# OpenGene/repaq

Measured on AMD Instinct MI355X. Metric: raw FASTQ MB/s encode+decode, higher is better.
Workload: dtype u8; 1 GPU; configs[2]: synthetic NovaSeq PE150 two files (-i/-I), 2 x 4.01 GB FASTQ (fqgen profile 1, 11200000 pairs, seed 3, N 20 ppm), -k 1000, encode + decode; chunks_per_gpu=3360, parity=unchecked (checked with --full)

## Files before the change

repaq_amd/csrc/dec/pos_lists.h:

```cpp
#pragma once
#define POS2_SEG 1024u
#define POS2_SEG_BIG 2048u
#define POS2_CELL 1024u
typedef uint16_t plist_t;
__device__ __forceinline__ uint32_t plist_pos(uint32_t e, uint32_t w0) { return e == 0xFFFFFFFFu ? e : w0 + ((e - w0) & 0xFFFFu); }
struct PosSrc { const uint8_t* sp; uint32_t slen; uint8_t q; };
__device__ __forceinline__ PosSrc pos_src_of(const uint8_t* __restrict__ img, const DChunk& d, const DevHeader* __restrict__ D, uint32_t jj, DecStatus* st) {
    PosSrc s; s.sp = nullptr; s.slen = 0; s.q = 0;
    const uint32_t nn = D->n_normal, hf = D->flags; const uint8_t* cp = img + d.off;
    if (jj == nn) { if (hf & H_N_POS) { s.sp = cp + d.o_npos; s.slen = d.npos_size; s.q = (uint8_t)'N'; } return s; }
    if (jj > nn || jj >= NPOS_SLOT || (hf & H_DONT_QUAL) || !(hf & H_QUAL_BY_COL)) return s;
    if (4ull * nn > d.qual_size) { if (st && lane_id() == 0) atomicOr(&st->err, (uint32_t)DE_CORRUPT); return s; }
    const uint8_t* qp = cp + d.o_qual; uint64_t off = 4ull * nn;
    for (uint32_t i = 0; i < jj; i++) off += ld_u32(qp + 4 * i);
    const uint32_t sl = ld_u32(qp + 4 * jj);
    if (off + sl > d.qual_size) { if (st && lane_id() == 0) atomicOr(&st->err, (uint32_t)DE_CORRUPT); return s; }
    s.sp = qp + off; s.slen = sl; s.q = D->normal[jj];
    return s;
}
__device__ __forceinline__ void pos_lane_adv_cnt(const PosFront& f, uint32_t slen, uint32_t i0, uint32_t st, int& adv, int& cnt) {
    adv = 0; cnt = 0;
#pragma unroll
    for (int k = 0; k < 4; k++) {
        const uint32_t b0 = f.bt[k]; const bool valid = i0 + (uint32_t)k < slen;
        const uint32_t b1 = (uint32_t)(f.v >> (8 * (k + 1))) & 0xFFu, b2 = (uint32_t)(f.v >> (8 * (k + 2))) & 0xFFu, b3 = (uint32_t)(f.v >> (8 * (k + 3))) & 0xFFu;
        if (valid && st == 0) {
            if ((b0 & 0x80u) == 0) { adv += (int)b0 + 1; cnt++; }
            else if ((b0 & 0x40u) == 0) { adv += (int)(((b0 & 0x3Fu) << 8) | b1) + 1; cnt++; }
            else if ((b0 & 0x20u) == 0) { adv += (int)(b0 & 0x1Fu) + 1; cnt += (int)(b0 & 0x1Fu) + 1; }
            else { adv += (int)(((b0 & 0x1Fu) << 24) | (b1 << 16) | (b2 << 8) | b3) + 1; cnt++; }
        }
        if (valid) st = fn_apply(f.fn[k], st);
    }
}
__device__ __forceinline__ int sel4(const int (&v)[4], uint32_t t) { return t == 0 ? v[0] : (t == 1 ? v[1] : (t == 2 ? v[2] : v[3])); }
__device__ __forceinline__ void pos_lane_adv_cnt4(const PosFront& f, uint32_t slen, uint32_t i0, int (&adv)[4], int (&cnt)[4]) {
    const uint32_t nv = i0 >= slen ? 0u : (slen - i0 < 4u ? slen - i0 : 4u);
    int ca[4], cc[4]; uint32_t tl[4];
#pragma unroll
    for (int k = 0; k < 4; k++) {
        const uint32_t b0 = f.bt[k];
        const uint32_t b1 = (uint32_t)(f.v >> (8 * (k + 1))) & 0xFFu, b2 = (uint32_t)(f.v >> (8 * (k + 2))) & 0xFFu, b3 = (uint32_t)(f.v >> (8 * (k + 3))) & 0xFFu;
        if ((b0 & 0x80u) == 0) { ca[k] = (int)b0 + 1; cc[k] = 1; tl[k] = 1; }
        else if ((b0 & 0x40u) == 0) { ca[k] = (int)(((b0 & 0x3Fu) << 8) | b1) + 1; cc[k] = 1; tl[k] = 2; }
        else if ((b0 & 0x20u) == 0) { ca[k] = (int)(b0 & 0x1Fu) + 1; cc[k] = ca[k]; tl[k] = 1; }
        else { ca[k] = (int)(((b0 & 0x1Fu) << 24) | (b1 << 16) | (b2 << 8) | b3) + 1; cc[k] = 1; tl[k] = 4; }
    }
#pragma unroll
    for (int k = 2; k >= 0; k--) {
        const uint32_t nx = (uint32_t)k + tl[k];
        if (nx < nv) { const int a_ = nx == 1u ? ca[1] : (nx == 2u ? ca[2] : ca[3]), c_ = nx == 1u ? cc[1] : (nx == 2u ? cc[2] : cc[3]); ca[k] += a_; cc[k] += c_; }
    }
#pragma unroll
    for (int s = 0; s < 4; s++) { const bool on = (uint32_t)s < nv; adv[s] = on ? ca[s] : 0; cnt[s] = on ? cc[s] : 0; }
}
#define POS_ADV_MAX 0x3FFFFFFFull
__device__ __forceinline__ int pos_adv_sat(int v) { return v > (int)POS_ADV_MAX ? (int)POS_ADV_MAX : v; }
__global__ void k_dec_pos_sum2(const uint8_t* __restrict__ img, const DChunk* __restrict__ CH, const DevHeader* __restrict__ D,
                               uint8_t* __restrict__ segF, int* __restrict__ segA, uint32_t* __restrict__ segN, uint32_t maxseg, DecStatus* st, uint64_t img_bytes, uint32_t jj0, uint32_t nstr,
                               uint32_t segb) {
    const uint32_t g = blockIdx.x * (blockDim.x >> 6) + (uint32_t)wave_id(), jj = jj0 + blockIdx.y, c = blockIdx.z; const int l = lane_id();
            const uint8_t* lim = img + img_bytes;
    const DChunk d = CH[c];
    const PosSrc s = pos_src_of(img, d, D, jj, g == 0 ? st : nullptr);
    if (g == 0 && l == 0) segN[(size_t)c * nstr + jj] = (s.slen + segb - 1) / segb;
    const uint32_t b0 = g * segb; if (b0 >= s.slen) return;
    const uint32_t b1 = b0 + segb < s.slen ? b0 + segb : s.slen;
    uint32_t Fcum = POS_ID; int a[4] = { 0, 0, 0, 0 }, n[4] = { 0, 0, 0, 0 };
    PosStep nxt = pos_fetch(s.sp, s.slen, b0 + 4u * (uint32_t)l, lim);
    for (uint32_t base = b0; base < b1; base += 256u) {
        const uint32_t i0 = base + 4u * (uint32_t)l;
        const PosStep w = nxt;
        if (base + 256u < b1) nxt = pos_fetch(s.sp, s.slen, i0 + 256u, lim);
        const PosFront f = pos_front(w, s.sp, s.slen, i0, l);
        const uint32_t Fex = wave_shr1(f.Fin, POS_ID);
        const uint32_t G = fn_compose(Fcum, Fex);
        int la[4], lc[4]; pos_lane_adv_cnt4(f, s.slen, i0, la, lc);
#pragma unroll
        for (int e = 0; e < 4; e++) { const uint32_t t_ = fn_apply(G, e); a[e] += sel4(la, t_); n[e] += sel4(lc, t_); }
        Fcum = fn_compose(Fcum, wave_last(f.Fin));
    }
#pragma unroll
    for (int e = 0; e < 4; e++) { const unsigned long long w64 = wave_sum<unsigned long long>((unsigned long long)(uint32_t)a[e]); a[e] = (int)(w64 > POS_ADV_MAX ? POS_ADV_MAX : w64);
            n[e] = wave_sum(n[e]); }
    if (l == 0) { const size_t idx = ((size_t)c * nstr + jj) * maxseg + g; segF[idx] = (uint8_t)fn_pack8(Fcum);
#pragma unroll
                  for (int e = 0; e < 4; e++) { segA[8 * idx + e] = a[e]; segA[8 * idx + 4 + e] = n[e]; } }
}
struct PosLink { uint32_t F; int a[4], n[4]; };
__device__ __forceinline__ PosLink poslink_then(const PosLink& x, const PosLink& y) {
    PosLink r; r.F = fn_compose(x.F, y.F);
#pragma unroll
    for (int s = 0; s < 4; s++) { const uint32_t t = fn_apply(x.F, s); r.a[s] = pos_adv_sat(x.a[s] + sel4(y.a, t)); r.n[s] = x.n[s] + sel4(y.n, t); }
    return r;
}
__device__ __forceinline__ PosLink poslink_shfl_up(const PosLink& v, unsigned dd) {
    PosLink u; u.F = __shfl_up(v.F, dd);
#pragma unroll
    for (int s = 0; s < 4; s++) { u.a[s] = __shfl_up(v.a[s], dd); u.n[s] = __shfl_up(v.n[s], dd); }
    return u;
}
__global__ void k_dec_pos_link2(const uint8_t* __restrict__ segF, const int* __restrict__ segA, const uint32_t* __restrict__ segN, uint8_t* __restrict__ segS,
        int* __restrict__ segP,
                                uint32_t* __restrict__ segK, uint32_t* __restrict__ nent, uint32_t maxseg, uint32_t n_streams,
                                const DChunk* __restrict__ CH, uint32_t nstr, DecStatus* st) {
    const uint32_t t = blockIdx.x * (blockDim.x >> 6) + (uint32_t)wave_id(); if (t >= n_streams) return;
    const int l = lane_id(); const uint32_t n = segN[t];
    uint32_t cs = 0; int cp = -1; uint32_t ck = 0;
    for (uint32_t base = 0; base < n; base += 64) {
        const uint32_t g = base + (uint32_t)l; const size_t idx = (size_t)t * maxseg + g;
        PosLink me; me.F = POS_ID;
#pragma unroll
        for (int s = 0; s < 4; s++) { me.a[s] = 0; me.n[s] = 0; }
        if (g < n) { me.F = fn_unpack8(segF[idx]);
#pragma unroll
                     for (int s = 0; s < 4; s++) { me.a[s] = segA[8 * idx + s]; me.n[s] = segA[8 * idx + 4 + s]; } }
        PosLink inc = me;
#pragma unroll
        for (int dd = 1; dd < 64; dd <<= 1) { const PosLink up = poslink_shfl_up(inc, (unsigned)dd); if (l >= dd) inc = poslink_then(up, inc); }
        PosLink ex = poslink_shfl_up(inc, 1u);
        if (l == 0) { ex.F = POS_ID;
#pragma unroll
                      for (int s = 0; s < 4; s++) { ex.a[s] = 0; ex.n[s] = 0; } }
        if (g < n) { segS[idx] = (uint8_t)(fn_apply(ex.F, cs)); segP[idx] = pos_adv_sat(cp + sel4(ex.a, cs)); segK[idx] = ck + (uint32_t)sel4(ex.n, cs); }
        const uint32_t Fl = wave_last(inc.F); int al[4], nl[4];
#pragma unroll
        for (int s = 0; s < 4; s++) { al[s] = wave_last(inc.a[s]); nl[s] = wave_last(inc.n[s]); }
        cp = pos_adv_sat(cp + sel4(al, cs)); ck += (uint32_t)sel4(nl, cs); cs = fn_apply(Fl, cs);
    }
    if (l == 0) {
        nent[t] = ck;
        const unsigned long long ext = CH[t / nstr].bases;
        if (cp >= 0 && (unsigned long long)cp >= ext + 32768ull) atomicOr(&st->err, (uint32_t)DE_LIST_ALIAS);
    }
}
__global__ void k_dec_pos_off(const uint32_t* __restrict__ nent, unsigned long long* __restrict__ loff, uint32_t n_streams, DecStatus* st) {
    const uint32_t K = (n_streams + blockDim.x - 1) / blockDim.x, i0 = threadIdx.x * K, i1 = i0 + K < n_streams ? i0 + K : n_streams;
    unsigned long long acc = 0;
    for (uint32_t i = i0; i < i1; i++) acc += nent[i];
    unsigned long long tot; unsigned long long run = block_excl_sum<unsigned long long>(acc, &tot);
    for (uint32_t i = i0; i < i1; i++) { loff[i] = run; run += nent[i]; }
    if (threadIdx.x == 0) st->list_need = tot;
}
__global__ void k_dec_pos_list(const uint8_t* __restrict__ img, const DChunk* __restrict__ CH, const DevHeader* __restrict__ D,
                               const uint8_t* __restrict__ segS, const int* __restrict__ segP, const uint32_t* __restrict__ segK, const unsigned long long* __restrict__ loff,
                               plist_t* __restrict__ plist, unsigned long long cap, uint32_t* __restrict__ cellidx, uint32_t maxseg, uint32_t ncell, uint64_t img_bytes, uint32_t jj0, uint32_t nstr, const DecStatus* st,
                               uint32_t segb) {
    if (st->list_need > cap) return;
    const uint32_t g = blockIdx.x * (blockDim.x >> 6) + (uint32_t)wave_id(), jj = jj0 + blockIdx.y, c = blockIdx.z; const int l = lane_id();
            const uint8_t* lim = img + img_bytes;
    const DChunk d = CH[c];
    const PosSrc s = pos_src_of(img, d, D, jj, nullptr);
    const uint32_t b0 = g * segb; if (b0 >= s.slen) return;
    const size_t t = (size_t)c * nstr + jj, idx = t * maxseg + g;
    uint32_t carry = segS[idx]; int last = segP[idx]; uint32_t k0 = segK[idx];
    plist_t* const out = plist + loff[t]; uint32_t* const cells = cellidx + t * ncell;
    const uint32_t b1 = b0 + segb < s.slen ? b0 + segb : s.slen;
    PosStep nxt = pos_fetch(s.sp, s.slen, b0 + 4u * (uint32_t)l, lim);
    for (uint32_t base = b0; base < b1; base += 256u) {
        const uint32_t i0 = base + 4u * (uint32_t)l;
        const PosStep w = nxt;
        if (base + 256u < b1) nxt = pos_fetch(s.sp, s.slen, i0 + 256u, lim);
        const PosFront f = pos_front(w, s.sp, s.slen, i0, l);
        const uint32_t Fex = wave_shr1(f.Fin, POS_ID);
        uint32_t st0 = fn_apply(Fex, carry);
        int adv[4]; uint32_t run[4]; bool start[4]; int lane_adv = 0, lane_cnt = 0;
#pragma unroll
        for (int k = 0; k < 4; k++) {
            const uint32_t bb = f.bt[k]; const bool valid = i0 + (uint32_t)k < s.slen;
            const uint32_t b1_ = (uint32_t)(f.v >> (8 * (k + 1))) & 0xFFu, b2_ = (uint32_t)(f.v >> (8 * (k + 2))) & 0xFFu, b3_ = (uint32_t)(f.v >> (8 * (k + 3))) & 0xFFu;
            start[k] = valid && st0 == 0; adv[k] = 0; run[k] = 0;
            if (start[k]) {
                if ((bb & 0x80u) == 0) adv[k] = (int)bb + 1;
                else if ((bb & 0x40u) == 0) adv[k] = (int)(((bb & 0x3Fu) << 8) | b1_) + 1;
                else if ((bb & 0x20u) == 0) { run[k] = (bb & 0x1Fu) + 1; adv[k] = (int)run[k]; }
                else adv[k] = (int)(((bb & 0x1Fu) << 24) | (b1_ << 16) | (b2_ << 8) | b3_) + 1;
                lane_cnt += run[k] ? (int)run[k] : 1;
            }
            lane_adv += adv[k];
            if (valid) st0 = fn_apply(f.fn[k], st0);
        }
        const int ia = wave_incl_sum(lane_adv), ic = wave_incl_sum(lane_cnt);
        int end = last + ia - lane_adv; uint32_t k = k0 + (uint32_t)(ic - lane_cnt);
#pragma unroll
        for (int q = 0; q < 4; q++) {
            if (!start[q]) continue;
            const int prev = end; end += adv[q];
            const int lo = run[q] ? end - (int)run[q] + 1 : end;
            int pp = prev;
            for (int p = lo; p <= end; p++, k++) {
                out[k] = (plist_t)p;
                uint32_t c0 = pp < 0 ? 0u : (uint32_t)pp / POS2_CELL + 1u; const uint32_t c1 = (uint32_t)p / POS2_CELL;
                for (; c0 <= c1 && c0 < ncell; c0++) cells[c0] = k;
                pp = p;
            }
        }
        last += wave_last(ia); k0 += (uint32_t)wave_last(ic); carry = fn_apply((uint32_t)wave_last(f.Fin), carry);
    }
}

__global__ void k_dec_except(const uint8_t* __restrict__ img, const DChunk* __restrict__ CH, const DevHeader* __restrict__ D, DReadTab R,
                             const uint64_t* __restrict__ qbase, uint8_t* __restrict__ qdec) {
    const uint32_t c = blockIdx.y, nn = D->n_normal, hf = D->flags;
    const DChunk d = CH[c]; const uint8_t* qp = img + d.off + d.o_qual; const uint32_t f = d.rbase;
    const uint32_t len = R.pq[f + d.reads] - R.pq[f]; uint8_t* dst = qdec + qbase[c];
    const uint32_t t = blockIdx.x * blockDim.x + threadIdx.x, NT = gridDim.x * blockDim.x;
    if (hf & H_DONT_QUAL) { for (uint32_t i = t; i < d.qual_size && i < len; i += NT) dst[i] = qp[i]; return; }
    if (!(hf & H_QUAL_BY_COL) || 4ull * nn > d.qual_size) return;
    uint64_t off = 4ull * nn;
    for (uint32_t i = 0; i < nn; i++) off += ld_u32(qp + 4 * i);
    if (off > d.qual_size) return;
    const uint32_t nrec = (uint32_t)((d.qual_size - off) / 5);
    for (uint32_t i = t; i < nrec; i += NT) { const uint8_t* r = qp + off + 5ull * i; const uint32_t pos = ld_u32(r + 1); if (pos < len) dst[pos] = r[0]; }
}
__global__ void k_dec_rle(const uint8_t* __restrict__ img, const DChunk* __restrict__ CH, const DevHeader* __restrict__ D, DReadTab R,
                          const uint64_t* __restrict__ qbase, uint8_t* __restrict__ qdec) {
    __shared__ uint8_t s_b2q[256]; __shared__ uint32_t s_carry;
    const uint32_t c = blockIdx.y; const DChunk d = CH[c]; const uint8_t* qp = img + d.off + d.o_qual; const uint32_t f = d.rbase;
    const uint32_t len = R.pq[f + d.reads] - R.pq[f]; uint8_t* dst = qdec + qbase[c];
    const uint32_t bins = D->bytes[16]; int mx = (int)bins * 2 - 3; if (mx < 1) mx = 1;
    const uint32_t nq = mx >= 64 ? 1u : mx >= 32 ? 2u : mx >= 16 ? 3u : mx >= 8 ? 4u : mx >= 4 ? 5u : mx >= 2 ? 6u : 7u, mask = (1u << (8u - nq)) - 1u;
    for (uint32_t i = threadIdx.x; i < 256; i += blockDim.x) s_b2q[i] = 0;
    __syncthreads();
    for (uint32_t i = threadIdx.x; i < bins; i += blockDim.x) s_b2q[(uint8_t)(i ? 2u * i - 1u : 0u)] = D->bytes[17 + i];
    if (threadIdx.x == 0) s_carry = 0;
    __syncthreads();
    if (d.qual_size == 0 || len == 0) return;
    for (uint32_t rounds = 0; ; rounds++) {
        for (uint32_t b0 = 0; b0 < d.qual_size; b0 += blockDim.x) {
            const uint32_t i = b0 + threadIdx.x; uint32_t run = 0, q = 0;
            if (i < d.qual_size) { const uint32_t e = qp[i]; if ((e & 1u) == 0) { q = 0; run = (e >> 1) + 1u; } else { q = e & mask; run = (e >> (8u - nq)) + 1u; } }
            uint32_t tot; const uint32_t ex = block_excl_sum<uint32_t>(run, &tot);
            const uint32_t start = s_carry + ex; const uint8_t v = s_b2q[q];
            for (uint32_t p = start; p < start + run && p < len; p++) dst[p] = v;
            __syncthreads();
            if (threadIdx.x == 0) s_carry += tot;
            __syncthreads();
            if (s_carry >= len) return;
        }
    }
}
__global__ void k_dec_fill(uint8_t* __restrict__ p, uint64_t n, const DevHeader* __restrict__ D) {
    const uint32_t v = D->major & 0xFFu; const uint4 q = make_uint4(v * 0x01010101u, v * 0x01010101u, v * 0x01010101u, v * 0x01010101u);
    uint4* p4 = (uint4*)p; const uint64_t n4 = n / 16;
    for (uint64_t i = (uint64_t)blockIdx.x * blockDim.x + threadIdx.x; i < n4; i += (uint64_t)gridDim.x * blockDim.x) p4[i] = q;
    if (blockIdx.x == 0 && threadIdx.x < (n & 15u)) p[n4 * 16 + threadIdx.x] = (uint8_t)v;
}

__global__ void k_dec_coords(const uint8_t* __restrict__ img, const DChunk* __restrict__ CH, const DevHeader* __restrict__ D, uint32_t* __restrict__ xv,
        uint32_t* __restrict__ yv) {
    const uint32_t axis = blockIdx.x, c = blockIdx.y;
    if (!(D->flags & (axis ? H_Y : H_X))) return;
    const DChunk d = CH[c]; const uint8_t* sp = img + d.off + (axis ? d.o_y : d.o_x) + 4; const uint32_t slen = axis ? d.y_size : d.x_size;
    const uint32_t num = (d.flags & C_PE_INTERLEAVED) ? d.reads / 2 : d.reads;
    uint32_t* out = (axis ? yv : xv) + d.rbase;
    const int l = lane_id(); uint32_t carry = 0, cur = 1000u, produced = 0;
    auto fetch = [&](uint32_t base_) -> uint32_t { const uint32_t i_ = base_ + (uint32_t)l; return i_ < slen ? (uint32_t)sp[i_] : 0u; };
    uint32_t w1 = fetch(0u), w2 = fetch(64u);
    for (uint32_t base = 0; base < slen; base += 64) {
        const uint32_t i = base + (uint32_t)l; const bool valid = i < slen;
        const uint32_t b0 = w1; w1 = w2; w2 = fetch(base + 128u);
        const uint32_t n0 = wave_read(w1, 0u), n1 = wave_read(w1, 1u);
        uint32_t b1 = (uint32_t)__shfl_down((int)b0, 1u), b2 = (uint32_t)__shfl_down((int)b0, 2u);
        if (l == 63) { b1 = n0; b2 = n1; } else if (l == 62) b2 = n0;
        const uint32_t tl = (b0 & 0x80u) == 0 ? 2u : ((b0 & 0xE0u) == 0xE0u ? 3u : 1u);
        const uint32_t before = wave_token_states(tl, valid, carry);
        const bool start = valid && before == 0;
        uint32_t cnt = 0, isabs = 0, val = 0;
        if (start) {
            if ((b0 & 0x80u) == 0) { isabs = 1; val = (b0 << 8) | b1; cnt = 1; }
            else if ((b0 & 0x40u) == 0) { val = (b0 & 0x3Fu) + 1; cnt = 1; }
            else if ((b0 & 0x20u) == 0) { val = 0; cnt = (b0 & 0x1Fu) + 1; }
            else { isabs = 1; val = ((b0 & 0x1Fu) << 16) | (b1 << 8) | b2; cnt = 1; }
        }
        uint32_t v = val, a = isabs;
#pragma unroll
        for (int dd = 1; dd < 64; dd <<= 1) { const uint32_t tv = __shfl_up(v, (unsigned)dd), ta = __shfl_up(a, (unsigned)dd); if (l >= dd && !a) { v += tv; a = ta; } }
        const uint32_t value = a ? v : cur + v;
        const uint32_t incl = wave_incl_sum(cnt); const uint32_t o = produced + incl - cnt;
        if (start) for (uint32_t k = 0; k < cnt; k++) if (o + k < num) out[o + k] = value;
        produced += wave_last(incl); cur = wave_last(value);
    }
}
```

repaq_amd/csrc/rfq_api.hip:

```cpp
#include "rfq_ctx.h"
#include <cstring>
#include <algorithm>
#include <new>
#include <cstdlib>
#include <string>
#include <cerrno>

extern "C" const char* rfq_version(void) {
#ifdef RFQ_SIMT_EMULATION
    return "rfq_hip 0.1.0 simt-emulation (test build, not a product path)";
#else
    return "rfq_hip 0.1.0 gfx950";
#endif
}

static bool opt_num(const std::string& v, long long lo, long long hi, long long* out) {
    if (v.empty()) return false;
    errno = 0; char* end = nullptr; const long long x = strtoll(v.c_str(), &end, 10);
    if (errno || !end || *end || end == v.c_str() || x < lo || x > hi) return false;
    *out = x; return true;
}
extern "C" int rfq_set_option(rfq_ctx* c, const char* name, const char* value) {
    if (!c || !name) return RFQ_E_ARG;
    const std::string n = name, v = value ? value : ""; const bool set = !v.empty(); const RfqOpts d; long long num = 0;
#define RFQ_OPT_NUM(LO, HI, WHAT) if (set && !opt_num(v, LO, HI, &num)) return rfq_fail(c, RFQ_E_ARG, "%s is " WHAT " (got \"%s\")", name, v.c_str());
    if (n == "RFQ_GATHER") { if (set && v != "old" && v != "tile") return rfq_fail(c, RFQ_E_ARG, "RFQ_GATHER is old or tile"); c->opt.gather_old = v == "old"; }
    else if (n == "RFQ_QUAL") { if (set && v != "bytes" && v != "masks") return rfq_fail(c, RFQ_E_ARG, "RFQ_QUAL is bytes or masks"); c->opt.qual_bytes = v == "bytes"; }
    else if (n == "RFQ_CODER") { if (set && v != "list" && v != "mask") return rfq_fail(c, RFQ_E_ARG, "RFQ_CODER is list or mask");
            c->opt.coder = v == "list" ? 1 : (v == "mask" ? 2 : 0); }
    else if (n == "RFQ_INDEX") { if (set && v != "2pass" && v != "1pass") return rfq_fail(c, RFQ_E_ARG, "RFQ_INDEX is 2pass or 1pass"); c->opt.index_2pass = v == "2pass"; }
    else if (n == "RFQ_IDX_TILES") { if (set && v != "4" && v != "8" && v != "16") return rfq_fail(c, RFQ_E_ARG, "RFQ_IDX_TILES is 4, 8 or 16");
            c->opt.idx_tiles = set ? atoi(v.c_str()) : d.idx_tiles; }
    else if (n == "RFQ_STREAMS") { if (set && v != "1" && v != "2") return rfq_fail(c, RFQ_E_ARG, "RFQ_STREAMS is 1 or 2"); c->opt.one_stream = v == "1"; }
    else if (n == "RFQ_SLICE_BYTES") { RFQ_OPT_NUM(1024, 0xFFFFFFF0ll - 16, "a number of bytes in 1024 .. 2^32 - 32") c->opt.slice_bytes = set ? (size_t)num : 0; }
    else if (n == "RFQ_SLICE_BASES") { RFQ_OPT_NUM(1, 0xFFFFFFF0ll, "a number of bases in 1 .. 2^32 - 16") c->opt.slice_bases = set ? (uint64_t)num : 0; }
    else if (n == "RFQ_WALK") { if (set && v != "exact" && v != "guess") return rfq_fail(c, RFQ_E_ARG, "RFQ_WALK is guess or exact"); c->opt.walk_exact = v == "exact"; }
    else if (n == "RFQ_GW_SHIFT") { RFQ_OPT_NUM(4, 30, "4 .. 30") c->opt.gw_shift = set ? (int)num : d.gw_shift; }
    else if (n == "RFQ_MATERIALISE") { if (set && v != "0" && v != "1") return rfq_fail(c, RFQ_E_ARG, "RFQ_MATERIALISE is 0 or 1"); c->opt.materialise = v == "1"; }
    else if (n == "RFQ_TRACE") { if (set && v != "0" && v != "1") return rfq_fail(c, RFQ_E_ARG, "RFQ_TRACE is 0 or 1"); c->opt.trace = v == "1"; }
    else if (n == "RFQ_G2_PAD") { RFQ_OPT_NUM(0, 150000, "0 .. 150000 bytes of LDS") c->opt.g2_pad = set ? (uint32_t)num : 0u; }
    else if (n == "RFQ_SP_PAD") { RFQ_OPT_NUM(0, 150000, "0 .. 150000 bytes of LDS") c->opt.sp_pad = set ? (uint32_t)num : d.sp_pad; }
    else if (n == "RFQ_POS_SEG") { if (set && v != "1024" && v != "2048") return rfq_fail(c, RFQ_E_ARG, "RFQ_POS_SEG is 1024 or 2048"); c->opt.pos_seg = set ? atoi(v.c_str()) : 0; }
    else if (n == "RFQ_SPEC") { if (set && v != "0" && v != "1") return rfq_fail(c, RFQ_E_ARG, "RFQ_SPEC is 0 or 1"); c->opt.no_spec = v == "0"; }
    else return rfq_fail(c, RFQ_E_ARG, "unknown option %s", name);
#undef RFQ_OPT_NUM
    return RFQ_OK;
}
static const char* const RFQ_OPTION_NAMES[] = { "RFQ_GATHER", "RFQ_QUAL", "RFQ_CODER", "RFQ_INDEX", "RFQ_IDX_TILES", "RFQ_STREAMS", "RFQ_SLICE_BYTES", "RFQ_SLICE_BASES", "RFQ_WALK", "RFQ_GW_SHIFT", "RFQ_MATERIALISE", "RFQ_TRACE", "RFQ_G2_PAD", "RFQ_SP_PAD", "RFQ_POS_SEG", "RFQ_SPEC" };
extern "C" const char* rfq_option_name(int i) { return (i >= 0 && i < (int)(sizeof RFQ_OPTION_NAMES / sizeof RFQ_OPTION_NAMES[0])) ? RFQ_OPTION_NAMES[i] : nullptr; }
extern "C" int rfq_get_option(const rfq_ctx* c, const char* name, char* out, size_t cap) {
    if (!c || !name || !out || !cap) return RFQ_E_ARG;
    const std::string n = name; const RfqOpts& o = c->opt; const RfqOpts d; std::string v;
    if (n == "RFQ_GATHER") v = o.gather_old ? "old" : "";
    else if (n == "RFQ_QUAL") v = o.qual_bytes ? "bytes" : "";
    else if (n == "RFQ_CODER") v = o.coder == 1 ? "list" : (o.coder == 2 ? "mask" : "");
    else if (n == "RFQ_INDEX") v = o.index_2pass ? "2pass" : "";
    else if (n == "RFQ_IDX_TILES") v = o.idx_tiles != d.idx_tiles ? std::to_string(o.idx_tiles) : "";
    else if (n == "RFQ_STREAMS") v = o.one_stream ? "1" : "";
    else if (n == "RFQ_SLICE_BYTES") v = o.slice_bytes ? std::to_string(o.slice_bytes) : "";
    else if (n == "RFQ_SLICE_BASES") v = o.slice_bases ? std::to_string(o.slice_bases) : "";
    else if (n == "RFQ_WALK") v = o.walk_exact ? "exact" : "";
    else if (n == "RFQ_GW_SHIFT") v = o.gw_shift != d.gw_shift ? std::to_string(o.gw_shift) : "";
    else if (n == "RFQ_MATERIALISE") v = o.materialise ? "1" : "";
    else if (n == "RFQ_TRACE") v = o.trace ? "1" : "";
    else if (n == "RFQ_G2_PAD") v = o.g2_pad ? std::to_string(o.g2_pad) : "";
    else if (n == "RFQ_SP_PAD") v = o.sp_pad != d.sp_pad ? std::to_string(o.sp_pad) : "";
    else if (n == "RFQ_POS_SEG") v = o.pos_seg ? std::to_string(o.pos_seg) : "";
    else if (n == "RFQ_SPEC") v = o.no_spec ? "0" : "";
    else return RFQ_E_ARG;
    if (v.size() + 1 > cap) return RFQ_E_NOSPACE;
    memcpy(out, v.c_str(), v.size() + 1);
    return RFQ_OK;
}

extern "C" int rfq_create(rfq_ctx** out, int device_id) {
    if (!out) return RFQ_E_ARG;
    *out = nullptr;
    int n = 0;
    if (hipGetDeviceCount(&n) != hipSuccess || n <= 0) return RFQ_E_NO_DEVICE;
    if (device_id < 0 || device_id >= n) return RFQ_E_NO_DEVICE;
    if (hipSetDevice(device_id) != hipSuccess) return RFQ_E_NO_DEVICE;
    rfq_ctx* c = new (std::nothrow) rfq_ctx();
    if (!c) return RFQ_E_HIP;
    c->device = device_id;
    { int cu = 0; if (hipDeviceGetAttribute(&cu, hipDeviceAttributeMultiprocessorCount, device_id) == hipSuccess && cu > 0) c->n_cu = (uint32_t)cu; }
    if (hipStreamCreate(&c->stream) != hipSuccess) { delete c; return RFQ_E_NO_DEVICE; }
    c->own_stream = true;
    memset(&c->h_hdr, 0, sizeof c->h_hdr);
    for (const char* nm : RFQ_OPTION_NAMES) { const char* v = getenv(nm); if (v && *v && rfq_set_option(c, nm, v) != RFQ_OK) fprintf(stderr, "rfq_hip: ignoring %s=%s (%s)\n", nm, v, c->err.c_str()); }
    c->err.clear();
    *out = c;
    return RFQ_OK;
}

extern "C" void rfq_destroy(rfq_ctx* c) {
    if (!c) return;
    (void)hipSetDevice(c->device);
    (void)hipDeviceSynchronize();
    for (auto& b : c->b) b.release();
    c->d_hdr.release(); c->d_status.release(); c->d_cmp.release(); c->out_img.release(); c->out_fq1.release(); c->out_fq2.release(); c->out_acc.release();
            c->out_acc1.release(); c->out_acc2.release();
    c->timer.destroy();
    if (c->copy) { (void)hipStreamDestroy(c->copy); for (auto& e : c->copy_ev) if (e) (void)hipEventDestroy(e); }
    if (c->own_stream && c->stream) (void)hipStreamDestroy(c->stream);
    if (c->pin) (void)hipHostFree(c->pin);
    if (c->pin_up) (void)hipHostFree(c->pin_up);
    if (c->ev_up) (void)hipEventDestroy(c->ev_up);
    if (c->aux) (void)hipStreamDestroy(c->aux);
    if (c->ev_fork) (void)hipEventDestroy(c->ev_fork);
    if (c->ev_join) (void)hipEventDestroy(c->ev_join);
    if (c->ev_mid) (void)hipEventDestroy(c->ev_mid);
    if (c->aux2) (void)hipStreamDestroy(c->aux2);
    if (c->ev_f) (void)hipEventDestroy(c->ev_f);
    delete c;
}

extern "C" const char* rfq_last_error(const rfq_ctx* c) { return c ? c->err.c_str() : "null context"; }

extern "C" int rfq_set_stream(rfq_ctx* c, void* s) {
    if (!c) return RFQ_E_ARG;
    if (s) {
        if (c->own_stream && c->stream) (void)hipStreamDestroy(c->stream);
        c->stream = (hipStream_t)s; c->own_stream = false;
    } else if (!c->own_stream) {
        if (hipStreamCreate(&c->stream) != hipSuccess) return rfq_fail(c, RFQ_E_HIP, "hipStreamCreate failed");
        c->own_stream = true;
    }
    return RFQ_OK;
}

int rfq_upload_header(rfq_ctx* c, const uint8_t* h, size_t n);

extern "C" int rfq_set_header(rfq_ctx* c, const uint8_t* h, size_t n) {
    if (!c || !h) return RFQ_E_ARG;
    c->err.clear();
    return rfq_upload_header(c, h, n);
}
extern "C" int rfq_get_header(rfq_ctx* c, uint8_t* out, size_t* len) {
    if (!c || !out || !len) return RFQ_E_ARG;
    if (!c->have_hdr) return rfq_fail(c, RFQ_E_STATE, "no header has been made or set on this context");
    memcpy(out, c->h_hdr.bytes, c->h_hdr.len); *len = c->h_hdr.len;
    return RFQ_OK;
}
extern "C" void rfq_clear_header(rfq_ctx* c) { if (c) { c->have_hdr = false; c->hdr_on_device = false; c->dense_ok = false; c->e3_pieces_failed = false; c->mixed_lengths = false; memset(&c->h_hdr, 0, sizeof c->h_hdr); } }

extern "C" int rfq_last_timings(const rfq_ctx* c, const char** names, float* ms, int cap) {
    if (!c) return 0;
    int n = 0;
    for (size_t i = 0; i < c->timer.ms.size() && n < cap; i++, n++) { if (names) names[n] = c->timer.names[i]; if (ms) ms[n] = c->timer.ms[i]; }
    return n;
}

extern "C" int rfq_dev_malloc(rfq_ctx* c, void** p, size_t n) {
    if (!c || !p) return RFQ_E_ARG;
    HIPCHK(c, hipSetDevice(c->device));
    HIPCHK(c, hipMalloc(p, n ? n : 256));
    return RFQ_OK;
}
extern "C" int rfq_dev_free(rfq_ctx* c, void* p) { if (!c) return RFQ_E_ARG; if (p) HIPCHK(c, hipFree(p)); return RFQ_OK; }
extern "C" int rfq_copy_h2d(rfq_ctx* c, void* d, const void* h, size_t n) {
    if (!c) return RFQ_E_ARG;
    HIPCHK(c, hipSetDevice(c->device));
    if (n) { HIPCHK(c, hipMemcpyAsync(d, h, n, hipMemcpyHostToDevice, c->stream)); HIPCHK(c, hipStreamSynchronize(c->stream)); }
    return RFQ_OK;
}
extern "C" int rfq_copy_h2d_async(rfq_ctx* c, void* d, const void* h, size_t n, uint64_t* ticket) {
    if (!c) return RFQ_E_ARG;
    HIPCHK(c, hipSetDevice(c->device));
    if (!c->copy) HIPCHK(c, hipStreamCreateWithFlags(&c->copy, hipStreamNonBlocking));
    const uint64_t t = c->copy_next; hipEvent_t& ev = c->copy_ev[t & 63u];
    if (t >= 64 && c->copy_done + 64 <= t) { HIPCHK(c, hipEventSynchronize(ev)); c->copy_done = t - 63; }
    if (!ev) HIPCHK(c, hipEventCreateWithFlags(&ev, hipEventDisableTiming));
    if (n) HIPCHK(c, hipMemcpyAsync(d, h, n, hipMemcpyHostToDevice, c->copy));
    HIPCHK(c, hipEventRecord(ev, c->copy));
    c->copy_next = t + 1;
    if (ticket) *ticket = t;
    return RFQ_OK;
}
extern "C" int rfq_copy_done(rfq_ctx* c, uint64_t ticket) {
    if (!c || ticket >= c->copy_next) return RFQ_E_ARG;
    if (ticket < c->copy_done || ticket + 64 < c->copy_next) return 1;
    const hipError_t e = hipEventQuery(c->copy_ev[ticket & 63u]);
    if (e == hipSuccess) return 1;
    if (e == hipErrorNotReady) { (void)hipGetLastError(); return 0; }
    return rfq_fail(c, RFQ_E_HIP, "hipEventQuery failed: %s", hipGetErrorString(e));
}
extern "C" int rfq_copy_sync(rfq_ctx* c) {
    if (!c) return RFQ_E_ARG;
    if (c->copy) { HIPCHK(c, hipSetDevice(c->device)); HIPCHK(c, hipStreamSynchronize(c->copy)); c->copy_done = c->copy_next; }
    return RFQ_OK;
}
extern "C" int rfq_copy_d2d(rfq_ctx* c, void* dst, const void* src, size_t n) {
    if (!c) return RFQ_E_ARG;
    HIPCHK(c, hipSetDevice(c->device));
    if (n) { HIPCHK(c, hipMemcpyAsync(dst, src, n, hipMemcpyDeviceToDevice, c->stream)); HIPCHK(c, hipStreamSynchronize(c->stream)); }
    return RFQ_OK;
}
extern "C" int rfq_copy_peer(rfq_ctx* c, void* dst, const rfq_ctx* src_ctx, const void* src, size_t n) {
    if (!c || !src_ctx) return RFQ_E_ARG;
    HIPCHK(c, hipSetDevice(c->device));
    if (n) {
        if (src_ctx->device == c->device) HIPCHK(c, hipMemcpyAsync(dst, src, n, hipMemcpyDeviceToDevice, c->stream));
        else HIPCHK(c, hipMemcpyPeerAsync(dst, c->device, src, src_ctx->device, n, c->stream));
        HIPCHK(c, hipStreamSynchronize(c->stream));
    }
    return RFQ_OK;
}
__global__ __launch_bounds__(256) void k_first_diff(const uint8_t* __restrict__ a, const uint8_t* __restrict__ b, uint64_t n, unsigned long long* __restrict__ out) {
    const uint64_t tid = (uint64_t)blockIdx.x * blockDim.x + threadIdx.x, stride = (uint64_t)gridDim.x * blockDim.x;
    unsigned long long best = ~0ull;
    if (((((uintptr_t)a) | ((uintptr_t)b)) & 15) == 0) {
        const uint64_t n16 = n >> 4;
        const uint4* a4 = (const uint4*)a; const uint4* b4 = (const uint4*)b;
        for (uint64_t i = tid; i < n16; i += stride) {
            const uint4 x = a4[i], y = b4[i];
            const uint32_t d[4] = { x.x ^ y.x, x.y ^ y.y, x.z ^ y.z, x.w ^ y.w };
            if (d[0] | d[1] | d[2] | d[3]) {
                for (int w = 0; w < 4; w++) if (d[w]) { best = i * 16 + w * 4 + ((__ffs((int)d[w]) - 1) >> 3); break; }
                break;
            }
        }
        if (tid == 0) for (uint64_t i = n16 << 4; i < n; i++) if (a[i] != b[i]) { if (i < best) best = i; break; }
    } else {
        for (uint64_t i = tid; i < n; i += stride) if (a[i] != b[i]) { best = i; break; }
    }
    if (best != ~0ull) atomicMin(out, best);
}
extern "C" int rfq_compare_bytes(rfq_ctx* c, const void* d_a, const void* d_b, size_t n, uint64_t* first_diff) {
    if (!c || !first_diff || (n && (!d_a || !d_b))) return RFQ_E_ARG;
    HIPCHK(c, hipSetDevice(c->device));
    *first_diff = n;
    if (!n) return RFQ_OK;
    HIPCHK(c, c->d_cmp.ensure(8));
    unsigned long long init = ~0ull, got = 0;
    HIPCHK(c, hipMemcpyAsync(c->d_cmp.p, &init, 8, hipMemcpyHostToDevice, c->stream));
    const uint64_t items = (n >> 4) + 1;
    const unsigned blocks = (unsigned)std::min<uint64_t>((items + 255) / 256, 256u * 16u);
    hipLaunchKernelGGL(k_first_diff, dim3(blocks), dim3(256), 0, c->stream, (const uint8_t*)d_a, (const uint8_t*)d_b, (uint64_t)n, c->d_cmp.as<unsigned long long>());
    KCHK(c, "k_first_diff");
    HIPCHK(c, hipMemcpyAsync(&got, c->d_cmp.p, 8, hipMemcpyDeviceToHost, c->stream));
    HIPCHK(c, hipStreamSynchronize(c->stream));
    if (got != ~0ull) *first_diff = (uint64_t)got;
    return RFQ_OK;
}
extern "C" int rfq_host_alloc(rfq_ctx* c, void** p, size_t n) {
    if (!c || !p) return RFQ_E_ARG;
    HIPCHK(c, hipSetDevice(c->device));
    HIPCHK(c, hipHostMalloc(p, n ? n : 256, 0));
    return RFQ_OK;
}
extern "C" int rfq_host_free(rfq_ctx* c, void* p) { if (!c) return RFQ_E_ARG; if (p) HIPCHK(c, hipHostFree(p)); return RFQ_OK; }
extern "C" int rfq_host_register(rfq_ctx* c, void* h_ptr, size_t n) {
    if (!c || !h_ptr || !n) return RFQ_E_ARG;
    HIPCHK(c, hipSetDevice(c->device));
    HIPCHK(c, hipHostRegister(h_ptr, n, hipHostRegisterDefault));
    return RFQ_OK;
}
extern "C" int rfq_host_unregister(rfq_ctx* c, void* h_ptr) {
    if (!c || !h_ptr) return RFQ_E_ARG;
    HIPCHK(c, hipHostUnregister(h_ptr));
    return RFQ_OK;
}
extern "C" int rfq_copy_d2h(rfq_ctx* c, void* h, const void* d, size_t n) {
    if (!c) return RFQ_E_ARG;
    HIPCHK(c, hipSetDevice(c->device));
    if (n) { HIPCHK(c, hipMemcpyAsync(h, d, n, hipMemcpyDeviceToHost, c->stream)); HIPCHK(c, hipStreamSynchronize(c->stream)); }
    return RFQ_OK;
}

__global__ void k_selftest_wave(const unsigned long long* __restrict__ in, unsigned long long* __restrict__ out) {
    const uint32_t i = blockIdx.x * 64u + threadIdx.x; const unsigned long long v = in[i];
    const uint32_t a = (uint32_t)v; const int sa = (int)a;
    unsigned long long* o = out + 12ull * i;
    o[0] = wave_incl_sum<uint32_t>(a);
    o[1] = wave_incl_sum<unsigned long long>(v);
    o[2] = (unsigned long long)(long long)wave_incl_max<int>(sa);
    o[3] = (unsigned long long)wave_incl_max<long long>((long long)v);
    o[4] = wave_sum<uint32_t>(a);
    o[5] = wave_min<uint32_t>(a);
    o[6] = wave_max<uint32_t>(a);
    o[7] = ((unsigned long long)wave_and(a) << 32) | wave_or(a);
    o[8] = wave_shr1<uint32_t>(a, 0xABCD1234u);
    o[9] = wave_last<uint32_t>(a);
    o[10] = wave_min<unsigned long long>(v);
    { U4 u; u.a = a; u.b = a >> 3; u.c = a ^ 0x5A5Au; u.d = (uint32_t)(v >> 32); const U4 r = wave_incl_sum(u);
            o[11] = ((unsigned long long)(r.a + r.b + r.c) << 32) | r.d; }
}
extern "C" int rfq_selftest_wave(rfq_ctx* c, const uint64_t* h_in, uint32_t n_waves, uint64_t* h_out) {
    if (!c || !h_in || !h_out || !n_waves) return RFQ_E_ARG;
    HIPCHK(c, hipSetDevice(c->device));
    const size_t n = (size_t)n_waves * 64u;
    void *din = nullptr, *dout = nullptr;
    HIPCHK(c, hipMalloc(&din, n * 8)); if (hipMalloc(&dout, n * 96) != hipSuccess) { (void)hipFree(din); return rfq_fail(c, RFQ_E_HIP, "hipMalloc failed"); }
    hipError_t e = hipMemcpy(din, h_in, n * 8, hipMemcpyHostToDevice);
    if (e == hipSuccess) { hipLaunchKernelGGL(k_selftest_wave, dim3(n_waves), dim3(64), 0, c->stream, (const unsigned long long*)din, (unsigned long long*)dout);
            e = hipGetLastError(); }
    if (e == hipSuccess) e = hipStreamSynchronize(c->stream);
    if (e == hipSuccess) e = hipMemcpy(h_out, dout, n * 96, hipMemcpyDeviceToHost);
    (void)hipFree(din); (void)hipFree(dout);
    if (e != hipSuccess) return rfq_fail(c, RFQ_E_HIP, "rfq_selftest_wave: %s", hipGetErrorString(e));
    return RFQ_OK;
}
```

repaq_amd/csrc/rfq_ctx.h:

```cpp
#pragma once
#include "rfq_common.h"
#include "../../include/rfq_hip.h"
#include <cstring>
#include <string>
#include <vector>
#include <cstdio>
#include <cstdarg>
#include <algorithm>

struct DBuf {
    void* p = nullptr; size_t cap = 0;
    hipError_t ensure(size_t n) {
        if (n <= cap) return hipSuccess;
        if (p) { (void)hipFree(p); p = nullptr; cap = 0; }
        size_t want = n + n / 4 + 4096;
        hipError_t e = hipMalloc(&p, want);
        if (e != hipSuccess) { p = nullptr; return e; }
        cap = want; return hipSuccess;
    }
    hipError_t ensure_keep(size_t n, size_t keep, hipStream_t s) {
        if (n <= cap) return hipSuccess;
        void* q = nullptr; const size_t want = n + n / 2 + 4096;
        hipError_t e = hipMalloc(&q, want);
        if (e != hipSuccess) return e;
        if (p && keep) { e = hipMemcpyAsync(q, p, keep, hipMemcpyDeviceToDevice, s); if (e == hipSuccess) e = hipStreamSynchronize(s);
                if (e != hipSuccess) { (void)hipFree(q); return e; } }
        if (p) (void)hipFree(p);
        p = q; cap = want; return hipSuccess;
    }
    void release() { if (p) (void)hipFree(p); p = nullptr; cap = 0; }
    template <class T> T* as() const { return (T*)p; }
};

struct StageTimer {
    struct Stage { const char* name; hipEvent_t a, b; };
    std::vector<Stage> stages; size_t used = 0; std::vector<float> ms; std::vector<const char*> names;
    void reset() { used = 0; }
    void begin(const char* name, hipStream_t s) {
        if (used == stages.size()) { Stage st; st.name = name; (void)hipEventCreate(&st.a); (void)hipEventCreate(&st.b); stages.push_back(st); }
        stages[used].name = name; (void)hipEventRecord(stages[used].a, s);
    }
    void end(hipStream_t s) { (void)hipEventRecord(stages[used].b, s); used++; }
    void collect() {
        ms.assign(used, 0.f); names.assign(used, nullptr);
        for (size_t i = 0; i < used; i++) { (void)hipEventElapsedTime(&ms[i], stages[i].a, stages[i].b); names[i] = stages[i].name; }
    }
    void destroy() { for (auto& s : stages) { (void)hipEventDestroy(s.a); (void)hipEventDestroy(s.b); } stages.clear(); }
};
struct StageSums {
    std::vector<std::pair<const char*, float>> v;
    void add(const StageTimer& t) {
        for (size_t i = 0; i < t.names.size(); i++) {
            auto q = std::find_if(v.begin(), v.end(), [&](const std::pair<const char*, float>& e) { return e.first == t.names[i]; });
            if (q == v.end()) v.emplace_back(t.names[i], t.ms[i]); else q->second += t.ms[i];
        }
    }
    void publish(StageTimer& t) const { t.names.clear(); t.ms.clear(); for (auto& q : v) { t.names.push_back(q.first); t.ms.push_back(q.second); } }
};

static inline uint32_t grid_x_for(uint32_t n_chunks, uint32_t tiles_per_chunk, uint32_t slots) {
    uint32_t best = 1; double best_eff = 0.0;
    if (!n_chunks || !slots) return 1;
    for (uint32_t k = 6; k <= 12; k++) {
        uint32_t bx = (uint32_t)(((uint64_t)k * slots + n_chunks / 2) / n_chunks);
        bx = std::max<uint32_t>(1u, std::min<uint32_t>(std::max<uint32_t>(bx, 1u), tiles_per_chunk));
        const double rounds = (double)bx * n_chunks / slots, full = (double)(uint64_t)(rounds + 0.999999), eff = full > 0 ? rounds / full : 0.0;
        if (eff > best_eff + 1e-3) { best = bx; best_eff = eff; }
    }
    return best;
}
struct RfqOpts {
    int  coder = 0;
    bool qual_bytes = false;
    bool gather_old = false;
    bool index_2pass = false;
    int  idx_tiles = 0;
    bool one_stream = false;
    size_t slice_bytes = 0;
    uint64_t slice_bases = 0;
    bool walk_exact = false;
    int  gw_shift = 16;
    bool materialise = false;
    bool trace = false;
    uint32_t g2_pad = 0;
    uint32_t sp_pad = 0;
    bool no_spec = false;
    int  pos_seg = 0;
};
struct rfq_ctx {
    RfqOpts opt;
    bool e3_pieces_failed = false;
    int device = 0; uint32_t n_cu = 256;
    hipStream_t stream = nullptr; bool own_stream = false;
    hipStream_t aux = nullptr; hipEvent_t ev_fork = nullptr, ev_join = nullptr, ev_mid = nullptr;
    hipStream_t aux2 = nullptr; hipEvent_t ev_f = nullptr;
    hipEvent_t ev_ovl = nullptr;
    hipStream_t copy = nullptr; hipEvent_t copy_ev[64] = {}; uint64_t copy_next = 0, copy_done = 0;
    bool aux_ready() {
        if (aux) return true;
        if (hipStreamCreateWithFlags(&aux, hipStreamNonBlocking) != hipSuccess) { aux = nullptr; return false; }
        if (hipEventCreateWithFlags(&ev_fork, hipEventDisableTiming) != hipSuccess || hipEventCreateWithFlags(&ev_join, hipEventDisableTiming) != hipSuccess ||
            hipEventCreateWithFlags(&ev_mid, hipEventDisableTiming) != hipSuccess) return false;
        if (hipStreamCreateWithFlags(&aux2, hipStreamNonBlocking) != hipSuccess) { aux2 = nullptr; return false; }
        if (hipEventCreateWithFlags(&ev_f, hipEventDisableTiming) != hipSuccess) return false;
        if (hipEventCreateWithFlags(&ev_ovl, hipEventDisableTiming) != hipSuccess) return false;
        return true;
    }
    std::string err;
    uint8_t* pin = nullptr; size_t pin_cap = 0, pin_used = 0;
    struct Pend { void* host; size_t off, n; }; std::vector<Pend> pend;
    hipError_t fetch(void* host, const void* dev, size_t n, hipStream_t s) {
        if (!n) return hipSuccess;
        if (!pin) { if (hipHostMalloc((void**)&pin, 1 << 16, 0) != hipSuccess) { pin = nullptr; (void)hipGetLastError(); } else pin_cap = 1 << 16; }
        const size_t off = (pin_used + 15) & ~(size_t)15;
        if (!pin || off + n > pin_cap) return hipMemcpyAsync(host, dev, n, hipMemcpyDeviceToHost, s);
        pend.push_back(Pend{ host, off, n }); pin_used = off + n;
        return hipMemcpyAsync(pin + off, dev, n, hipMemcpyDeviceToHost, s);
    }
    hipError_t fetch_sync(hipStream_t s) {
        const hipError_t e = hipStreamSynchronize(s);
        if (e == hipSuccess) for (const Pend& q : pend) memcpy(q.host, pin + q.off, q.n);
        pend.clear(); pin_used = 0;
        return e;
    }
    DBuf d_hdr;
    DevHeader h_hdr; bool have_hdr = false;
    bool hdr_on_device = false; uint8_t* pin_up = nullptr; hipEvent_t ev_up = nullptr; bool ev_up_pending = false;
    DBuf d_status; DevStatus h_status;
    DBuf d_cmp;
    DBuf b[120];
    DBuf out_img, out_fq1, out_fq2, out_acc, out_acc1, out_acc2;
    double rec_per_byte = 0.0; bool lazy_block = false;
    bool retried_room = false;
    bool mixed_lengths = false;
    bool dense_ok = false;
    bool qplane_dirty = true;
    uint32_t qplane_nd = 0, qplane_mask = 0;
    size_t qplane_stride = 0;
    std::vector<uint64_t> chunk_off;
    std::vector<uint64_t> scan_end[2];
    StageTimer timer;
};

static inline int rfq_fail(rfq_ctx* c, int code, const char* fmt, ...) {
    char buf[1024]; va_list ap; va_start(ap, fmt); vsnprintf(buf, sizeof buf, fmt, ap); va_end(ap);
    if (c) c->err = buf;
    return code;
}
#define HIPCHK(ctx, call) do { hipError_t e_ = (call); if (e_ != hipSuccess) return rfq_fail(ctx, RFQ_E_HIP, "%s failed: %s", #call, hipGetErrorString(e_)); } while (0)
#define KCHK(ctx, what) do { hipError_t e_ = hipGetLastError(); if (e_ != hipSuccess) return rfq_fail(ctx, RFQ_E_HIP, "launch of %s failed: %s", what, hipGetErrorString(e_)); } while (0)

#define SCAN_TPB 256
#define SCAN_ITEMS 8
#define SCAN_TILE (SCAN_TPB * SCAN_ITEMS)

template <class T> __global__ void k_scan_reduce(const T* __restrict__ in, T* __restrict__ partial, uint64_t n, const uint32_t* __restrict__ skip) {
    if (skip && *skip) return;
    const uint64_t base = (uint64_t)blockIdx.x * SCAN_TILE + (uint64_t)threadIdx.x;
    T v[SCAN_ITEMS];
#pragma unroll
    for (int i = 0; i < SCAN_ITEMS; i++) v[i] = base + (uint64_t)i * SCAN_TPB < n ? in[base + (uint64_t)i * SCAN_TPB] : T();
    T acc = T();
#pragma unroll
    for (int i = 0; i < SCAN_ITEMS; i++) acc = acc + v[i];
    T tot; (void)block_excl_sum<T>(acc, &tot);
    if (threadIdx.x == 0) partial[blockIdx.x] = tot;
}
template <class T> __global__ void k_scan_partials(T* __restrict__ partial, uint32_t nb, T* __restrict__ grand, const uint32_t* __restrict__ skip) {
    if (skip && *skip) return;
    const uint32_t K = (nb + SCAN_TPB - 1) / SCAN_TPB, i0 = threadIdx.x * K, i1 = i0 + K < nb ? i0 + K : nb;
    T acc = T();
    for (uint32_t i = i0; i < i1; i++) acc = acc + partial[i];
    T tot; T run = block_excl_sum<T>(acc, &tot);
    for (uint32_t i = i0; i < i1; i++) { const T v = partial[i]; partial[i] = run; run = run + v; }
    if (threadIdx.x == 0 && grand) *grand = tot;
}
template <class T> __global__ void k_scan_apply(const T* __restrict__ in, T* __restrict__ out, const T* __restrict__ partial, uint64_t n, int write_total, const uint32_t* __restrict__ skip) {
    if (skip && *skip) return;
    const uint64_t base = (uint64_t)blockIdx.x * SCAN_TILE + (uint64_t)threadIdx.x * SCAN_ITEMS;
    T v[SCAN_ITEMS]; T acc = T();
    for (int i = 0; i < SCAN_ITEMS; i++) { v[i] = base + i < n ? in[base + i] : T(); acc = acc + v[i]; }
    T tot; T ex = block_excl_sum<T>(acc, &tot);
    T run = partial[blockIdx.x] + ex;
    for (int i = 0; i < SCAN_ITEMS; i++) { if (base + i < n) out[base + i] = run; run = run + v[i]; }
    if (write_total && base < n && base + SCAN_ITEMS >= n) out[n] = run;
}
#define SCAN_SMALL 16384u
template <class T> __global__ void k_scan_small(const T* in, T* out, uint32_t n, int write_total, const uint32_t* __restrict__ skip) {
    if (skip && *skip) return;
    const uint32_t K = (n + SCAN_TPB - 1) / SCAN_TPB, i0 = threadIdx.x * K, i1 = i0 + K < n ? i0 + K : n;
    T acc = T();
    for (uint32_t i = i0; i < i1; i++) acc = acc + in[i];
    T tot; T run = block_excl_sum<T>(acc, &tot);
    for (uint32_t i = i0; i < i1; i++) { const T v = in[i]; out[i] = run; run = run + v; }
    if (write_total && threadIdx.x == 0) out[n] = tot;
}
template <class T> static inline void scan_exclusive(hipStream_t s, const T* in, T* out, uint64_t n, T* tmp, int write_total, const uint32_t* skip = nullptr) {
    if (n == 0) { if (write_total) (void)hipMemsetAsync(out, 0, sizeof(T), s); return; }
    if (n <= SCAN_SMALL) { hipLaunchKernelGGL((k_scan_small<T>), dim3(1), dim3(SCAN_TPB), 0, s, in, out, (uint32_t)n, write_total, skip); return; }
    const uint32_t nb = (uint32_t)((n + SCAN_TILE - 1) / SCAN_TILE);
    hipLaunchKernelGGL((k_scan_reduce<T>), dim3(nb), dim3(SCAN_TPB), 0, s, in, tmp, n, skip);
    hipLaunchKernelGGL((k_scan_partials<T>), dim3(1), dim3(SCAN_TPB), 0, s, tmp, nb, (T*)nullptr, skip);
    hipLaunchKernelGGL((k_scan_apply<T>), dim3(nb), dim3(SCAN_TPB), 0, s, in, out, (const T*)tmp, n, write_total, skip);
}

#define CLEAR_MAX 8
struct ClearList { uint32_t* p[CLEAR_MAX]; uint64_t words[CLEAR_MAX]; uint32_t val[CLEAR_MAX]; uint32_t n;
    void add(void* p_, size_t bytes, uint32_t v) { p[n] = (uint32_t*)p_; words[n] = (bytes + 3) / 4; val[n] = v; n++; } };
template <int UNUSED> __global__ void k_clear_list(ClearList z) {
    const uint64_t t0 = (uint64_t)blockIdx.x * blockDim.x + threadIdx.x, NT = (uint64_t)gridDim.x * blockDim.x;
    for (uint32_t r = 0; r < z.n; r++) {
        uint32_t* const p = z.p[r]; const uint32_t v = z.val[r]; const uint64_t n4 = z.words[r] >> 2;
        for (uint64_t i = t0; i < n4; i += NT) ((uint4*)p)[i] = make_uint4(v, v, v, v);
        for (uint64_t i = (n4 << 2) + t0; i < z.words[r]; i += NT) p[i] = v;
    }
}
static inline void clear_list(hipStream_t s, const ClearList& z) {
    size_t words = 0; for (uint32_t i = 0; i < z.n; i++) words = std::max<size_t>(words, (size_t)z.words[i]);
    if (z.n) hipLaunchKernelGGL((k_clear_list<0>), dim3((uint32_t)std::min<size_t>(2048, words / 1024 + 1)), dim3(256), 0, s, z);
}
```

repaq_amd/csrc/rfq_decode.hip:

```cpp
#include "rfq_ctx.h"
#include "rfq_decode_kernels.h"
#include <algorithm>
#include <cstring>
#include <cstdlib>

int rfq_upload_header(rfq_ctx* c, const uint8_t* h, size_t n);

enum DecBuf {
    DB_CHUNKS = 80, DB_STATUS, DB_LEN, DB_CHUNKID, DB_OV, DB_PVIN, DB_PV, DB_PQ, DB_TIN, DB_TP, DB_QBASE, DB_SBASE, DB_QDEC, DB_SDEC, DB_XV, DB_YV, DB_SCAN, DB_MID, DB_SEGF, DB_SEGA, DB_SEGN, DB_SEGS, DB_SEGP, DB_OFFT, DB_CELL, DB_SEGK, DB_NENT, DB_LOFF, DB_PLIST, DB_GWCAND, DB_GWLIST, DB_GWCNT, DB_GWLAND, DB_PQL, DB_PVL, DB_TPL, DB_CTEXT, DB_TBASE, DB_SDL, DB_END
};
static_assert(DB_END <= 120, "rfq_ctx::b too small");

#define RFQ_RANGE_TOO_BIG 2
struct DecRange { const DChunk* CH; uint32_t n_chunks, n_reads, max_reads, max_stream, max_npos, max_len, max_bases, max_nrec, max_one, pieces, piece_avg, piece_n1;
        uint64_t bases; };
static int dec_table_expanded(rfq_ctx* ctx, const rfq_decode_args* a, const DecRange& g, DReadTab& R, bool text, uint32_t* total_bases, U4* pv_tot) {
    hipStream_t S = ctx->stream; DBuf* B = ctx->b; const DevHeader* D = ctx->d_hdr.as<DevHeader>(); DecStatus* dst = B[DB_STATUS].as<DecStatus>();
    const uint32_t n_chunks = g.n_chunks, n_reads = g.n_reads, max_reads = std::max(g.max_reads, 1u);
    const size_t nr = (size_t)n_reads + 2, nc = (size_t)n_chunks + 2;
    HIPCHK(ctx, B[DB_CHUNKID].ensure(nr * 4));
    HIPCHK(ctx, B[DB_PVIN].ensure(nr * 16)); HIPCHK(ctx, B[DB_PV].ensure(nr * 16)); HIPCHK(ctx, B[DB_PQ].ensure(nr * 4));
    if (text) { HIPCHK(ctx, B[DB_TIN].ensure(nr * 16)); HIPCHK(ctx, B[DB_TP].ensure(nr * 16)); }
    HIPCHK(ctx, B[DB_QBASE].ensure(nc * 8)); HIPCHK(ctx, B[DB_SBASE].ensure(nc * 8));
    HIPCHK(ctx, B[DB_SCAN].ensure((nr / SCAN_TILE + 2) * 16 + 1024));
    R.chunk = B[DB_CHUNKID].as<uint32_t>();
    R.pvin = B[DB_PVIN].as<U4>(); R.pv = B[DB_PV].as<U4>(); R.pq = B[DB_PQ].as<uint32_t>();
    R.tin = text ? B[DB_TIN].as<U4>() : nullptr; R.tp = text ? B[DB_TP].as<U4>() : nullptr;
    hipLaunchKernelGGL(k_dec_readtab, dim3((max_reads + 255) / 256, n_chunks), dim3(256), 0, S, a->d_rfq, g.CH, D, R, dst);
    KCHK(ctx, "k_dec_readtab");
    scan_exclusive<uint32_t>(S, R.len, R.pq, n_reads, B[DB_SCAN].as<uint32_t>(), 1);
    scan_exclusive<U4>(S, R.pvin, R.pv, n_reads, B[DB_SCAN].as<U4>(), 1);
    HIPCHK(ctx, ctx->fetch(total_bases, R.pq + n_reads, 4, S));
    HIPCHK(ctx, ctx->fetch(pv_tot, R.pv + n_reads, 16, S));
    DecStatus h2; HIPCHK(ctx, ctx->fetch(&h2, dst, sizeof h2, S)); HIPCHK(ctx, ctx->fetch_sync(S));
    ctx->timer.end(S);
    if (h2.err & DE_CORRUPT) return rfq_fail(ctx, RFQ_E_FORMAT, "corrupt overlap buffer");
    return RFQ_OK;
}
struct DecExpanded { uint64_t* qbase; uint64_t* sbase; uint8_t* qdec; uint8_t* sdec; size_t qbytes, sbytes; };
static int dec_streams_expanded(rfq_ctx* ctx, const rfq_decode_args* a, const DecRange& g, const DReadTab& R, uint32_t total_bases, const U4& pv_tot, bool coords,
                                DecExpanded* E) {
    hipStream_t S = ctx->stream; DBuf* B = ctx->b; const DevHeader& HH = ctx->h_hdr; const DevHeader* D = ctx->d_hdr.as<DevHeader>();
    DecStatus* dst = B[DB_STATUS].as<DecStatus>(); const DChunk* CH = g.CH; const uint32_t n_chunks = g.n_chunks; const size_t nc = (size_t)n_chunks + 2;
    const bool rle_h = !(HH.flags & (H_DONT_QUAL | H_QUAL_BY_COL));
    ctx->timer.begin("streams", S);
    const size_t qbytes = (size_t)total_bases + 64 * nc + 256, sbytes = (size_t)pv_tot.d + 64 * nc + 256;
    HIPCHK(ctx, B[DB_QDEC].ensure(qbytes)); HIPCHK(ctx, B[DB_SDEC].ensure(sbytes));
    uint64_t* const qbase = B[DB_QBASE].as<uint64_t>(); uint64_t* const sbase = B[DB_SBASE].as<uint64_t>();
    uint8_t* const qdec = B[DB_QDEC].as<uint8_t>(); uint8_t* const sdec = B[DB_SDEC].as<uint8_t>();
    hipLaunchKernelGGL(k_dec_bases, dim3((n_chunks + 255) / 256), dim3(256), 0, S, CH, R, qbase, sbase, n_chunks);
    const bool forked = ctx->aux_ready();
    hipStream_t A = forked ? ctx->aux : S;
    if (forked) { HIPCHK(ctx, hipEventRecord(ctx->ev_fork, S)); HIPCHK(ctx, hipStreamWaitEvent(A, ctx->ev_fork, 0)); }
    const uint32_t bpc = std::max(1u, std::min(64u, 4096u / n_chunks));
    hipStream_t F = forked ? ctx->aux2 : S;
    if (forked) HIPCHK(ctx, hipStreamWaitEvent(F, ctx->ev_fork, 0));
    hipLaunchKernelGGL(k_dec_fill, dim3((uint32_t)std::min<size_t>(8192, (qbytes / 16 + 255) / 256 + 1)), dim3(256), 0, F, qdec, (uint64_t)qbytes, D);
    if (forked) HIPCHK(ctx, hipEventRecord(ctx->ev_f, F));
    if (coords) hipLaunchKernelGGL(k_dec_coords, dim3(2, n_chunks), dim3(64), 0, S, a->d_rfq, CH, D, B[DB_XV].as<uint32_t>(), B[DB_YV].as<uint32_t>());
    if ((HH.flags & H_N_POS) || ((HH.flags & H_QUAL_BY_COL) && !(HH.flags & H_DONT_QUAL))) {
        const bool bycol = (HH.flags & H_QUAL_BY_COL) && !(HH.flags & H_DONT_QUAL), hasn = (HH.flags & H_N_POS) != 0;
        const uint32_t nn = bycol ? std::min<uint32_t>(HH.n_normal, NPOS_SLOT) : 0u, nstr = HH.n_normal + 1;
        const uint32_t mq = nn ? g.max_stream / POS_SEG + 1 : 0u, mn = hasn ? g.max_npos / POS_SEG + 1 : 0u, maxseg = std::max(1u, std::max(mq, mn));
        const size_t nseg = (size_t)n_chunks * nstr * maxseg;
        HIPCHK(ctx, B[DB_SEGF].ensure(nseg + 16)); HIPCHK(ctx, B[DB_SEGA].ensure(nseg * 16 + 16)); HIPCHK(ctx, B[DB_SEGN].ensure((size_t)n_chunks * nstr * 4 + 16));
        HIPCHK(ctx, B[DB_SEGS].ensure(nseg + 16)); HIPCHK(ctx, B[DB_SEGP].ensure(nseg * 4 + 16));
        HIPCHK(ctx, hipMemsetAsync(B[DB_SEGN].p, 0, (size_t)n_chunks * nstr * 4, A));
#define RFQ_SUM_ARGS a->d_rfq, CH, D, R, (const uint64_t*)qbase, (const uint64_t*)sbase, qdec, sdec, B[DB_SEGF].as<uint8_t>(), B[DB_SEGA].as<int>(), B[DB_SEGN].as<uint32_t>(), maxseg, dst, (uint64_t)a->n
        if (nn) hipLaunchKernelGGL(k_dec_pos_sum, dim3(mq, nn, n_chunks), dim3(64), 0, A, RFQ_SUM_ARGS, 0u, nstr);
        if (hasn) hipLaunchKernelGGL(k_dec_pos_sum, dim3(mn, 1, n_chunks), dim3(64), 0, A, RFQ_SUM_ARGS, HH.n_normal, nstr);
#undef RFQ_SUM_ARGS
        hipLaunchKernelGGL(k_dec_pos_link, dim3((n_chunks * nstr + 255) / 256), dim3(256), 0, A, (const uint8_t*)B[DB_SEGF].as<uint8_t>(),
                (const int*)B[DB_SEGA].as<int>(),
                           (const uint32_t*)B[DB_SEGN].as<uint32_t>(), B[DB_SEGS].as<uint8_t>(), B[DB_SEGP].as<int>(), maxseg, n_chunks * nstr);
        if (forked) { HIPCHK(ctx, hipEventRecord(ctx->ev_mid, A)); HIPCHK(ctx, hipStreamWaitEvent(S, ctx->ev_mid, 0)); HIPCHK(ctx, hipStreamWaitEvent(S, ctx->ev_f, 0)); }
        hipLaunchKernelGGL(k_dec_unpack, dim3(bpc, n_chunks), dim3(256), 0, A, a->d_rfq, CH, R, (const uint64_t*)sbase, sdec, (uint64_t)a->n);
        if (nn) hipLaunchKernelGGL(k_dec_pos_emit, dim3(mq, nn, n_chunks), dim3(64), 0, S, a->d_rfq, CH, D, R, (const uint64_t*)qbase, (const uint64_t*)sbase, qdec, sdec,
                                   (const uint8_t*)B[DB_SEGS].as<uint8_t>(), (const int*)B[DB_SEGP].as<int>(), maxseg, (uint64_t)a->n, 0u, nstr);
        if (hasn) hipLaunchKernelGGL(k_dec_pos_emit, dim3(mn, 1, n_chunks), dim3(64), 0, A, a->d_rfq, CH, D, R, (const uint64_t*)qbase, (const uint64_t*)sbase, qdec,
                sdec,
                                     (const uint8_t*)B[DB_SEGS].as<uint8_t>(), (const int*)B[DB_SEGP].as<int>(), maxseg, (uint64_t)a->n, HH.n_normal, nstr);
    } else hipLaunchKernelGGL(k_dec_unpack, dim3(bpc, n_chunks), dim3(256), 0, A, a->d_rfq, CH, R, (const uint64_t*)sbase, sdec, (uint64_t)a->n);
    if (forked) { HIPCHK(ctx, hipEventRecord(ctx->ev_join, A)); HIPCHK(ctx, hipStreamWaitEvent(S, ctx->ev_join, 0)); HIPCHK(ctx, hipStreamWaitEvent(S, ctx->ev_f, 0)); }
    if (rle_h) hipLaunchKernelGGL(k_dec_rle, dim3(1, n_chunks), dim3(256), 0, S, a->d_rfq, CH, D, R, (const uint64_t*)qbase, qdec);
    hipLaunchKernelGGL(k_dec_except, dim3(bpc, n_chunks), dim3(256), 0, S, a->d_rfq, CH, D, R, (const uint64_t*)qbase, qdec);
    KCHK(ctx, "k_dec_streams");
    ctx->timer.end(S);
    E->qbase = qbase; E->sbase = sbase; E->qdec = qdec; E->sdec = sdec; E->qbytes = qbytes; E->sbytes = sbytes;
    return RFQ_OK;
}
struct FusedPlan { bool on; uint32_t e3k; bool n1big, shared_pieces; };
static FusedPlan plan_fused(const rfq_ctx* ctx, const DecRange& g, bool force_expanded) {
    const DevHeader& HH = ctx->h_hdr;
    const bool rle_h = !(HH.flags & (H_DONT_QUAL | H_QUAL_BY_COL));
    uint32_t e3k = 6; bool n1big = false;
    while (e3k >= 1 && ((uint64_t)g.max_len << e3k) > E3_QCAP) e3k--;
    if (g.pieces) {
        while (e3k >= 1 && ((uint64_t)g.piece_avg << e3k) > 204u) e3k--;
        const uint64_t need1 = ((uint64_t)g.piece_n1 << e3k) * 5u / 4u + 32u;
        if (need1 > ET_N1CAP) { if (e3k == 6 && need1 <= E3_N1BIG) n1big = true; else e3k = 0; }
    }
    const bool e3_ok = e3k >= (g.pieces ? 6u : 1u) && !(g.pieces && ctx->e3_pieces_failed);
    const bool on = !force_expanded && !ctx->opt.materialise && !rle_h && g.max_len <= 2000u && g.max_nrec <= 4096u && e3_ok && g.max_bases < (1u << 30) - 65536u;
    return { on, e3k, n1big, E3_SHARED_OK && !g.pieces && !(HH.flags & H_DONT_QUAL) };
}
struct ListChain { uint32_t maxseg = 1, ncell = 1, nstr = 1, mq = 0, mn = 0, nn = 0, segb = POS2_SEG; bool hasn = false, built = false, join = false; hipStream_t aux = nullptr; };
struct AuxJoin { rfq_ctx* c; bool armed; ~AuxJoin() { if (armed) (void)hipStreamSynchronize(c->aux); } };

static void launch_pos_list(rfq_ctx* ctx, const rfq_decode_args* a, const DecRange& g, const ListChain& L, hipStream_t LS) {
    DBuf* B = ctx->b; const DevHeader* D = ctx->d_hdr.as<DevHeader>(); const DecStatus* dst = B[DB_STATUS].as<DecStatus>();
    const unsigned long long cap = B[DB_PLIST].cap / sizeof(plist_t);
#define RFQ_LIST_ARGS a->d_rfq, g.CH, D, (const uint8_t*)B[DB_SEGS].as<uint8_t>(), (const int*)B[DB_SEGP].as<int>(), (const uint32_t*)B[DB_SEGK].as<uint32_t>(), \
                      (const unsigned long long*)B[DB_LOFF].as<unsigned long long>(), B[DB_PLIST].as<plist_t>(), cap, B[DB_CELL].as<uint32_t>(), L.maxseg, L.ncell, (uint64_t)a->n
    if (L.nn) hipLaunchKernelGGL(k_dec_pos_list, dim3((L.mq + 3) / 4, L.nn, g.n_chunks), dim3(256), 0, LS, RFQ_LIST_ARGS, 0u, L.nstr, dst, L.segb);
    if (L.hasn) hipLaunchKernelGGL(k_dec_pos_list, dim3((L.mn + 3) / 4, 1, g.n_chunks), dim3(256), 0, LS, RFQ_LIST_ARGS, ctx->h_hdr.n_normal, L.nstr, dst, L.segb);
#undef RFQ_LIST_ARGS
}
static int dec_list_chain(rfq_ctx* ctx, const rfq_decode_args* a, const DecRange& g, AuxJoin& guard, ListChain* L) {
    hipStream_t S = ctx->stream; DBuf* B = ctx->b; const DevHeader& HH = ctx->h_hdr; const DevHeader* D = ctx->d_hdr.as<DevHeader>();
    DecStatus* dst = B[DB_STATUS].as<DecStatus>(); const DChunk* CH = g.CH; const uint32_t n_chunks = g.n_chunks;
    const bool bycol_h = (HH.flags & H_QUAL_BY_COL) && !(HH.flags & H_DONT_QUAL);
    L->nstr = HH.n_normal + 1; L->hasn = (HH.flags & H_N_POS) != 0; L->nn = bycol_h ? std::min<uint32_t>(HH.n_normal, NPOS_SLOT) : 0u;
    if (!L->nn && !L->hasn) return RFQ_OK;
    const bool forked = ctx->aux_ready(); hipStream_t A = forked ? ctx->aux : S;
    if (forked) { HIPCHK(ctx, hipEventRecord(ctx->ev_fork, S)); HIPCHK(ctx, hipStreamWaitEvent(A, ctx->ev_fork, 0)); guard.armed = true; }
    L->segb = ctx->opt.pos_seg ? (uint32_t)ctx->opt.pos_seg : (std::max(g.max_one, g.max_npos) >= 32768u ? POS2_SEG_BIG : POS2_SEG);
    L->mq = L->nn ? g.max_one / L->segb + 1 : 0u; L->mn = L->hasn ? g.max_npos / L->segb + 1 : 0u; L->maxseg = std::max(1u, std::max(L->mq, L->mn));
    L->ncell = g.max_bases / POS2_CELL + 2;
    const size_t nst = (size_t)n_chunks * L->nstr, nseg = nst * L->maxseg, ncl = nst * L->ncell;
    HIPCHK(ctx, B[DB_SEGF].ensure(nseg + 16)); HIPCHK(ctx, B[DB_SEGA].ensure(nseg * 32 + 16)); HIPCHK(ctx, B[DB_SEGN].ensure(nst * 4 + 16));
    HIPCHK(ctx, B[DB_SEGS].ensure(nseg + 16)); HIPCHK(ctx, B[DB_SEGP].ensure(nseg * 4 + 16)); HIPCHK(ctx, B[DB_SEGK].ensure(nseg * 4 + 16));
    HIPCHK(ctx, B[DB_CELL].ensure(ncl * 4 + 16));
    HIPCHK(ctx, B[DB_NENT].ensure(nst * 4 + 16)); HIPCHK(ctx, B[DB_LOFF].ensure(nst * 8 + 16));
    if (B[DB_PLIST].ensure((size_t)(g.bases / 8 + 1024) * sizeof(plist_t)) != hipSuccess) { (void)hipGetLastError();
            HIPCHK(ctx, B[DB_PLIST].ensure((size_t)(g.bases / 32 + 1024) * sizeof(plist_t))); }
    { ClearList z; memset(&z, 0, sizeof z); z.add(B[DB_SEGN].p, nst * 4, 0u); z.add(B[DB_NENT].p, nst * 4, 0u); z.add(B[DB_CELL].p, ncl * 4, 0xFFFFFFFFu); clear_list(A, z); }
#define RFQ_SUM2_ARGS a->d_rfq, CH, D, B[DB_SEGF].as<uint8_t>(), B[DB_SEGA].as<int>(), B[DB_SEGN].as<uint32_t>(), L->maxseg, dst, (uint64_t)a->n
    if (L->nn) hipLaunchKernelGGL(k_dec_pos_sum2, dim3((L->mq + 3) / 4, L->nn, n_chunks), dim3(256), 0, A, RFQ_SUM2_ARGS, 0u, L->nstr, L->segb);
    if (L->hasn) hipLaunchKernelGGL(k_dec_pos_sum2, dim3((L->mn + 3) / 4, 1, n_chunks), dim3(256), 0, A, RFQ_SUM2_ARGS, HH.n_normal, L->nstr, L->segb);
#undef RFQ_SUM2_ARGS
    hipLaunchKernelGGL(k_dec_pos_link2, dim3((uint32_t)((nst + 3) / 4)), dim3(256), 0, A, (const uint8_t*)B[DB_SEGF].as<uint8_t>(), (const int*)B[DB_SEGA].as<int>(),
                       (const uint32_t*)B[DB_SEGN].as<uint32_t>(), B[DB_SEGS].as<uint8_t>(), B[DB_SEGP].as<int>(), B[DB_SEGK].as<uint32_t>(), B[DB_NENT].as<uint32_t>(),
                       L->maxseg, (uint32_t)nst, CH, L->nstr, dst);
    hipLaunchKernelGGL(k_dec_pos_off, dim3(1), dim3(256), 0, A, (const uint32_t*)B[DB_NENT].as<uint32_t>(), B[DB_LOFF].as<unsigned long long>(), (uint32_t)nst, dst);
    launch_pos_list(ctx, a, g, *L, A);
    L->built = true; L->join = forked; L->aux = A;
    KCHK(ctx, "k_dec_pos_*");
    return RFQ_OK;
}
static int dec_table_fused(rfq_ctx* ctx, const rfq_decode_args* a, const DecRange& g, const FusedPlan& P, const DReadTab& R, DFused* F) {
    hipStream_t S = ctx->stream; DBuf* B = ctx->b;
    const size_t nr = (size_t)g.n_reads + 2, nc = (size_t)g.n_chunks + 2;
    HIPCHK(ctx, B[DB_PQL].ensure((nr + nc) * 4)); HIPCHK(ctx, B[DB_TPL].ensure(nr * 8));
    if (!P.shared_pieces) HIPCHK(ctx, B[DB_PVL].ensure((nr + nc) * 16));
    HIPCHK(ctx, B[DB_CTEXT].ensure(nc * 16)); HIPCHK(ctx, B[DB_TBASE].ensure(nc * 16)); HIPCHK(ctx, B[DB_SCAN].ensure((nc / SCAN_TILE + 2) * 16 + 1024));
    HIPCHK(ctx, B[DB_SDL].ensure((nr + nc) * 4));
    U4* const pvl = P.shared_pieces ? (U4*)nullptr : B[DB_PVL].as<U4>();
    F->len = R.len; F->ov = R.ov; F->pql = B[DB_PQL].as<uint32_t>(); F->pvl = pvl; F->sdl = B[DB_SDL].as<uint32_t>();
    F->tpl = B[DB_TPL].as<uint2>(); F->tbase = B[DB_TBASE].as<U4>(); F->mid = R.mid;
    hipLaunchKernelGGL(k_dec_readtab2, dim3(g.n_chunks), dim3(256), 0, S, a->d_rfq, g.CH, ctx->d_hdr.as<DevHeader>(), R.len, R.ov, B[DB_PQL].as<uint32_t>(), pvl,
                       B[DB_SDL].as<uint32_t>(), B[DB_STATUS].as<DecStatus>());
    KCHK(ctx, "k_dec_readtab2");
    ctx->timer.end(S);
    return RFQ_OK;
}
static int dec_textlen_fused(rfq_ctx* ctx, const rfq_decode_args* a, const DecRange& g, const DReadTab& R) {
    hipStream_t S = ctx->stream; DBuf* B = ctx->b; const DevHeader* D = ctx->d_hdr.as<DevHeader>();
    ctx->timer.begin("streams", S);
    hipLaunchKernelGGL(k_dec_coords, dim3(2, g.n_chunks), dim3(64), 0, S, a->d_rfq, g.CH, D, B[DB_XV].as<uint32_t>(), B[DB_YV].as<uint32_t>());
    KCHK(ctx, "k_dec_coords");
    hipLaunchKernelGGL(k_dec_textlen2, dim3(g.n_chunks), dim3(256), 0, S, a->d_rfq, g.CH, D, (const uint32_t*)R.len, R.mid, (const uint32_t*)B[DB_XV].as<uint32_t>(),
                       (const uint32_t*)B[DB_YV].as<uint32_t>(), a->split_pe ? 1 : 0, B[DB_TPL].as<uint2>(), B[DB_CTEXT].as<U4>(), B[DB_STATUS].as<DecStatus>());
    KCHK(ctx, "k_dec_textlen2");
    scan_exclusive<U4>(S, B[DB_CTEXT].as<U4>(), B[DB_TBASE].as<U4>(), g.n_chunks, B[DB_SCAN].as<U4>(), 1);
    return RFQ_OK;
}
static void launch_emit3(rfq_ctx* ctx, const rfq_decode_args* a, const DecRange& g, const FusedPlan& P, const ListChain& L, const DFused& F,
                         uint8_t* o1, uint64_t cap1, uint8_t* o2, uint64_t cap2, unsigned long long list_cap) {
    DBuf* B = ctx->b; const bool hasn = (ctx->h_hdr.flags & H_N_POS) != 0;
    const uint32_t K = 1u << P.e3k, bx = grid_x_for(g.n_chunks, (std::max(g.max_reads, 1u) + K - 1) / K, (P.n1big ? 4u : 6u) * ctx->n_cu);
    const dim3 grid(bx, g.n_chunks);
#define RFQ_EMIT3_ARGS a->d_rfq, g.CH, ctx->d_hdr.as<DevHeader>(), F, (uint64_t)a->n, a->split_pe ? 1 : 0, o1, cap1, o2, cap2, B[DB_STATUS].as<DecStatus>(), \
                       (const plist_t*)B[DB_PLIST].as<plist_t>(), (const unsigned long long*)B[DB_LOFF].as<unsigned long long>(), (const uint32_t*)B[DB_NENT].as<uint32_t>(), \
                       (const uint32_t*)B[DB_CELL].as<uint32_t>(), L.ncell, L.nstr, P.e3k, list_cap
    if (P.n1big) {
        if (hasn) hipLaunchKernelGGL((k_dec_emit3<false, E3_N1BIG>), grid, dim3(256), 0, ctx->stream, RFQ_EMIT3_ARGS);
        else hipLaunchKernelGGL((k_dec_emit3<true, E3_N1BIG>), grid, dim3(256), 0, ctx->stream, RFQ_EMIT3_ARGS);
    } else if (F.pvl == nullptr) {
        if (hasn) hipLaunchKernelGGL((k_dec_emit3<false, ET_N1CAP, true>), grid, dim3(256), 0, ctx->stream, RFQ_EMIT3_ARGS);
        else hipLaunchKernelGGL((k_dec_emit3<true, ET_N1CAP, true>), grid, dim3(256), 0, ctx->stream, RFQ_EMIT3_ARGS);
    }
    else if (hasn) hipLaunchKernelGGL(k_dec_emit3<false>, grid, dim3(256), 0, ctx->stream, RFQ_EMIT3_ARGS);
    else hipLaunchKernelGGL(k_dec_emit3<true>, grid, dim3(256), 0, ctx->stream, RFQ_EMIT3_ARGS);
#undef RFQ_EMIT3_ARGS
}
static int decode_range(rfq_ctx* ctx, const rfq_decode_args* a, const DecRange& g, uint8_t* out1, uint64_t ocap1, uint8_t* out2, uint64_t ocap2,
                        uint8_t** p1, uint8_t** p2, size_t* n1, size_t* n2, uint64_t* nbases, bool force_expanded = false) {
    hipStream_t S = ctx->stream; DBuf* B = ctx->b; const DevHeader* D = ctx->d_hdr.as<DevHeader>();
    DecStatus* dst = B[DB_STATUS].as<DecStatus>(); DecStatus hs;
    const uint32_t n_chunks = g.n_chunks, n_reads = g.n_reads, max_reads = std::max(g.max_reads, 1u);
    const int split = a->split_pe ? 1 : 0;
    HIPCHK(ctx, hipMemsetAsync(dst, 0, sizeof(DecStatus), S));
    const FusedPlan P = plan_fused(ctx, g, force_expanded);
    ListChain L; AuxJoin aux_guard = { ctx, false };
    if (P.on) { const int rc = dec_list_chain(ctx, a, g, aux_guard, &L); if (rc) return rc; }
    ctx->timer.begin("read_table", S);
    const size_t nr = (size_t)n_reads + 2;
    HIPCHK(ctx, B[DB_LEN].ensure(nr * 4)); HIPCHK(ctx, B[DB_OV].ensure(nr * 4));
    HIPCHK(ctx, B[DB_XV].ensure(nr * 4)); HIPCHK(ctx, B[DB_YV].ensure(nr * 4)); HIPCHK(ctx, B[DB_MID].ensure(nr * 40));
    DReadTab R; memset(&R, 0, sizeof R); DFused F; memset(&F, 0, sizeof F); DecExpanded E; memset(&E, 0, sizeof E);
    R.len = B[DB_LEN].as<uint32_t>(); R.ov = B[DB_OV].as<int32_t>(); R.mid = B[DB_MID].as<uint8_t>();
    if (P.on) {
        int rc = dec_table_fused(ctx, a, g, P, R, &F);
        if (!rc) rc = dec_textlen_fused(ctx, a, g, R);
        if (rc) return rc;
        *nbases = g.bases;
    } else {
        uint32_t total_bases = 0; U4 pv_tot; memset(&pv_tot, 0, sizeof pv_tot);
        int rc = dec_table_expanded(ctx, a, g, R, true, &total_bases, &pv_tot);
        if (!rc) rc = dec_streams_expanded(ctx, a, g, R, total_bases, pv_tot, true, &E);
        if (rc) return rc;
        *nbases = total_bases;
        ctx->timer.begin("textlen", S);
        hipLaunchKernelGGL(k_dec_textlen, dim3((max_reads + 255) / 256, n_chunks), dim3(256), 0, S, a->d_rfq, g.CH, D, R, (const uint32_t*)B[DB_XV].as<uint32_t>(),
                           (const uint32_t*)B[DB_YV].as<uint32_t>(), split, dst);
        scan_exclusive<U4>(S, R.tin, R.tp, n_reads, B[DB_SCAN].as<U4>(), 1);
    }
    if (L.join) { HIPCHK(ctx, hipEventRecord(ctx->ev_join, L.aux)); HIPCHK(ctx, hipStreamWaitEvent(S, ctx->ev_join, 0)); }
    aux_guard.armed = false;
    bool emitted = P.on && L.built && out1 && (!a->split_pe || out2) && !((uintptr_t)out1 & 15u) && !(out2 && ((uintptr_t)out2 & 15u)) && !ctx->opt.no_spec;
    if (emitted) {
        ctx->timer.end(S);
        ctx->timer.begin("emit", S);
        launch_emit3(ctx, a, g, P, L, F, out1, ocap1, out2, ocap2, B[DB_PLIST].cap / sizeof(plist_t));
        KCHK(ctx, "k_dec_emit");
        ctx->timer.end(S);
    }
    U4 tt; HIPCHK(ctx, ctx->fetch(&tt, P.on ? B[DB_TBASE].as<U4>() + n_chunks : R.tp + n_reads, 16, S));
    uint8_t *o1, *o2;
    for (;;) {
        HIPCHK(ctx, ctx->fetch(&hs, dst, sizeof hs, S));
        HIPCHK(ctx, ctx->fetch_sync(S));
        if (hs.err & DE_CORRUPT_OV) return rfq_fail(ctx, RFQ_E_FORMAT, "corrupt overlap buffer");
        if (P.on && (hs.err & (DE_LIST_ALIAS | DE_E3_RETRY))) {
            if ((hs.err & DE_E3_RETRY) && g.pieces) ctx->e3_pieces_failed = true;
            return decode_range(ctx, a, g, out1, ocap1, out2, ocap2, p1, p2, n1, n2, nbases, true);
        }
        if (hs.err & DE_CORRUPT) return rfq_fail(ctx, RFQ_E_FORMAT, "corrupt quality buffer");
        if (L.built && hs.list_need > B[DB_PLIST].cap / sizeof(plist_t)) {
            if (emitted) { emitted = false; ctx->timer.begin("streams", S); }
            HIPCHK(ctx, B[DB_PLIST].ensure((size_t)(hs.list_need + 1024) * sizeof(plist_t)));
            launch_pos_list(ctx, a, g, L, S);
            KCHK(ctx, "k_dec_pos_list");
        }
        hs.text1 = hs.text2 = 0; for (int i = 0; i < 64; i++) { hs.text1 += hs.text_slots[0][i]; hs.text2 += hs.text_slots[1][i]; }
        if (hs.text1 >= 0xFFFFFFF0ull || hs.text2 >= 0xFFFFFFF0ull) return RFQ_RANGE_TOO_BIG;
        if ((out1 && ((uintptr_t)out1 & 15u)) || (out2 && ((uintptr_t)out2 & 15u))) return rfq_fail(ctx, RFQ_E_ARG, "output device pointers must be 16-byte aligned");
        uint64_t cap1, cap2;
        if (out1) { o1 = out1; cap1 = ocap1; } else { HIPCHK(ctx, ctx->out_fq1.ensure((size_t)tt.a + 64)); o1 = ctx->out_fq1.as<uint8_t>(); cap1 = ctx->out_fq1.cap; }
        if (out2) { o2 = out2; cap2 = ocap2; } else { HIPCHK(ctx, ctx->out_fq2.ensure((size_t)tt.b + 64)); o2 = ctx->out_fq2.as<uint8_t>(); cap2 = ctx->out_fq2.cap; }
        if (emitted) break;
        ctx->timer.end(S);
        ctx->timer.begin(P.on ? "emit" : "emit_expanded", S);
        if (P.on) launch_emit3(ctx, a, g, P, L, F, o1, cap1, o2, cap2, 0ull);
        else {
            const uint32_t bx = grid_x_for(n_chunks, (max_reads + ET_READS - 1) / ET_READS, 4u * ctx->n_cu);
            hipLaunchKernelGGL(k_dec_emit, dim3(bx, n_chunks), dim3(256), 0, S, a->d_rfq, g.CH, D, R, (const uint64_t*)E.qbase, (const uint64_t*)E.sbase,
                               (const uint8_t*)E.qdec, (const uint8_t*)E.sdec, (uint64_t)E.qbytes, (uint64_t)E.sbytes, (uint64_t)a->n, split, o1, cap1, o2, cap2, dst);
        }
        KCHK(ctx, "k_dec_emit");
        ctx->timer.end(S);
        emitted = true;
    }
    ctx->timer.collect();
    if (hs.err & (1u << 31)) return rfq_fail(ctx, RFQ_E_NOSPACE, "output buffer too small: need %u / %u bytes", tt.a, tt.b);
    *n1 = tt.a; *n2 = split ? tt.b : 0; *p1 = o1; *p2 = o2;
    return RFQ_OK;
}

static DecRange range_of(const DecStatus& hs, const DChunk* CH, uint32_t n_chunks, uint64_t reads, uint64_t bases) {
    DecRange g; g.CH = CH; g.n_chunks = n_chunks; g.n_reads = (uint32_t)reads; g.max_reads = hs.max_reads; g.max_stream = hs.max_stream;
            g.max_npos = hs.max_npos; g.max_len = hs.max_len; g.max_bases = hs.max_bases; g.max_nrec = hs.max_nrec; g.max_one = hs.max_one;
            g.pieces = hs.per_read_pieces; g.piece_avg = hs.piece_avg; g.piece_n1 = hs.piece_n1; g.bases = bases;
    return g;
}
struct ChunkSpan { uint32_t c0, c1; bool r1_only; };
static std::vector<ChunkSpan> plan_ranges(const std::vector<ChunkSpan>& pieces, const std::vector<DChunk>& hc, uint64_t slice_bases) {
    std::vector<ChunkSpan> fw, todo;
    for (auto& pc : pieces) {
        uint32_t c0 = pc.c0; uint64_t acc = 0, rd = 0;
        for (uint32_t c = pc.c0; c < pc.c1; c++) {
            if (c > c0 && (acc + hc[c].bases > slice_bases || rd + hc[c].reads > 0x7FFFFFF0ull)) { fw.push_back({ c0, c, pc.r1_only }); c0 = c; acc = 0; rd = 0; }
            acc += hc[c].bases; rd += hc[c].reads;
        }
        fw.push_back({ c0, pc.c1, pc.r1_only });
    }
    for (size_t i = fw.size(); i-- > 0;) todo.push_back(fw[i]);
    return todo;
}
static int span_range(rfq_ctx* ctx, const DecStatus& hs, DChunk* CHm, const std::vector<DChunk>& hc, const ChunkSpan& r, DecRange* g, uint64_t* reads) {
    uint64_t rd = 0, rbases = 0; for (uint32_t c = r.c0; c < r.c1; c++) { rd += hc[c].reads; rbases += hc[c].bases; }
    hipLaunchKernelGGL(k_dec_rebase, dim3((r.c1 - r.c0 + 255) / 256), dim3(256), 0, ctx->stream, CHm + r.c0, r.c1 - r.c0, hc[r.c0].rbase_abs);
    KCHK(ctx, "k_dec_rebase");
    *g = range_of(hs, CHm + r.c0, r.c1 - r.c0, rd, rbases); *reads = rd;
    return RFQ_OK;
}

static int dec_open(rfq_ctx* ctx, const rfq_decode_args* a, uint64_t* start) {
    HIPCHK(ctx, hipSetDevice(ctx->device));
    ctx->timer.reset();
    ctx->pend.clear(); ctx->pin_used = 0;
    *start = 0;
    if (a->has_header) {
        uint8_t hb[RFQ_HEADER_MAX]; const size_t take = std::min<size_t>(a->n, sizeof hb);
        if (take) HIPCHK(ctx, hipMemcpy(hb, a->d_rfq, take, hipMemcpyDeviceToHost));
        int rc = rfq_upload_header(ctx, hb, take);
        if (rc) return rc;
        *start = ctx->h_hdr.len;
    } else if (!ctx->have_hdr) return rfq_fail(ctx, RFQ_E_STATE, "decode without a header: pass has_header=1 or call rfq_set_header first");
    return RFQ_OK;
}
static int dec_walk(rfq_ctx* ctx, const rfq_decode_args* a, uint64_t start, DecStatus& hs) {
    hipStream_t S = ctx->stream; DBuf* B = ctx->b; const DevHeader& HH = ctx->h_hdr;
    if (HH.read_len_bytes != 1 && HH.read_len_bytes != 2 && HH.read_len_bytes != 4) return rfq_fail(ctx, RFQ_E_DATA,
            "header incorrect: read length bytes should be 1/2/4");
    const DevHeader* D = ctx->d_hdr.as<DevHeader>();

    ctx->timer.begin("walk", S);
    HIPCHK(ctx, B[DB_STATUS].ensure(sizeof(DecStatus)));
    DecStatus* dst = B[DB_STATUS].as<DecStatus>();
    uint32_t cap = (uint32_t)std::max<size_t>(B[DB_CHUNKS].cap / sizeof(DChunk), 4096);
    bool use_table = a->h_chunk_off && a->n_chunk_off && a->h_chunk_off[0] == start && a->h_chunk_off[a->n_chunk_off] <= a->n;
    bool guess = !use_table && !ctx->opt.walk_exact;
    for (;;) {
        if (use_table && a->n_chunk_off + 1u > cap) cap = a->n_chunk_off + 1u;
        HIPCHK(ctx, B[DB_CHUNKS].ensure((size_t)cap * sizeof(DChunk)));
        ClearList wz; memset(&wz, 0, sizeof wz); wz.add(dst, sizeof(DecStatus), 0u);
        const bool indexed = use_table || guess;
        if (use_table) {
            const size_t tb = ((size_t)a->n_chunk_off + 1) * 8;
            clear_list(S, wz);
            HIPCHK(ctx, B[DB_OFFT].ensure(tb));
            HIPCHK(ctx, hipMemcpyAsync(B[DB_OFFT].p, a->h_chunk_off, tb, hipMemcpyHostToDevice, S));
            hipLaunchKernelGGL(k_dec_table, dim3(1), dim3(256), 0, S, a->d_rfq, (uint64_t)a->n, (const uint64_t*)B[DB_OFFT].as<uint64_t>(), a->n_chunk_off,
                    B[DB_CHUNKS].as<DChunk>(), dst);
        } else if (guess) {
            HIPCHK(ctx, B[DB_OFFT].ensure(((size_t)cap + 2) * 8));
            HIPCHK(ctx, B[DB_GWCAND].ensure(GW_SEGS * 8 + 64)); HIPCHK(ctx, B[DB_GWLIST].ensure((size_t)GW_SEGS * GW_LCAP * 8));
                    HIPCHK(ctx, B[DB_GWCNT].ensure(GW_SEGS * 4 + 64)); HIPCHK(ctx, B[DB_GWLAND].ensure(GW_SEGS * 8 + 64));
            unsigned long long* cand = B[DB_GWCAND].as<unsigned long long>(); uint32_t* gbad = B[DB_GWCNT].as<uint32_t>() + GW_SEGS;
            wz.add(cand, GW_SEGS * 8, 0xFFFFFFFFu); wz.add(gbad, 4, 0u); clear_list(S, wz);
            const uint32_t mseg = (uint32_t)std::min<uint64_t>(GW_SEGS, std::max<uint64_t>(1, (a->n - start) >> ctx->opt.gw_shift));
            if (mseg > 1) hipLaunchKernelGGL(k_dec_gw_find, dim3(16, mseg - 1), dim3(256), 0, S, a->d_rfq, (uint64_t)a->n, start, D, cand, mseg);
            hipLaunchKernelGGL(k_dec_gw_walk, dim3(mseg), dim3(64), 0, S, a->d_rfq, (uint64_t)a->n, start, D, (const unsigned long long*)cand,
                    B[DB_GWLIST].as<unsigned long long>(), B[DB_GWCNT].as<uint32_t>(), B[DB_GWLAND].as<unsigned long long>(), gbad, mseg, a->final ? 1 : 0);
            hipLaunchKernelGGL(k_dec_gw_stitch, dim3(1), dim3(1024), 0, S, a->d_rfq, (uint64_t)a->n, start, D, (const unsigned long long*)cand,
                    (const unsigned long long*)B[DB_GWLIST].as<unsigned long long>(),
                               (const uint32_t*)B[DB_GWCNT].as<uint32_t>(), (const unsigned long long*)B[DB_GWLAND].as<unsigned long long>(), (const uint32_t*)gbad, B[DB_OFFT].as<uint64_t>(), cap, dst, mseg);
            hipLaunchKernelGGL(k_dec_table, dim3(1), dim3(256), 0, S, a->d_rfq, (uint64_t)a->n, (const uint64_t*)B[DB_OFFT].as<uint64_t>(), 0xFFFFFFFFu,
                    B[DB_CHUNKS].as<DChunk>(), dst);
        }
        else { clear_list(S, wz); hipLaunchKernelGGL(k_dec_walk, dim3(1), dim3(64), 0, S, a->d_rfq, (uint64_t)a->n, start, D, B[DB_CHUNKS].as<DChunk>(), cap, dst, a->final ? 1 : 0); }
        KCHK(ctx, "k_dec_walk");
        const uint32_t PARSE_AHEAD = use_table ? std::max(a->n_chunk_off, 1u) : 4096u;
        if (indexed) {
            hipLaunchKernelGGL(k_dec_parse, dim3(std::min(cap, PARSE_AHEAD)), dim3(64), 0, S, a->d_rfq, (uint64_t)a->n, D, B[DB_CHUNKS].as<DChunk>(), dst, 0u);
            hipLaunchKernelGGL(k_dec_summary, dim3(1), dim3(256), 0, S, (const DChunk*)B[DB_CHUNKS].as<DChunk>(), dst, 0u, std::min(cap, PARSE_AHEAD));
            KCHK(ctx, "k_dec_parse");
        }
        HIPCHK(ctx, ctx->fetch(&hs, dst, sizeof hs, S));
        HIPCHK(ctx, ctx->fetch_sync(S));
        if (use_table) {
            if (hs.pad || (hs.consumed != a->n && a->n - hs.consumed >= 18 && (a->final || hs.n_chunks == 0))) { use_table = false; guess = !ctx->opt.walk_exact;
                    continue; }
            break;
        }
        if (hs.overflow) { cap = hs.n_chunks + 1024; continue; }
        if (!indexed) { hs.max_nrec = 0xFFFFFFFFu; hs.max_one = hs.max_stream; hs.per_read_pieces = 1; hs.piece_avg = 0xFFFFu; hs.piece_n1 = 0xFFFFu; break; }
        if (hs.pad) { guess = false; continue; }
        if (hs.n_chunks > PARSE_AHEAD) {
            hipLaunchKernelGGL(k_dec_parse, dim3(hs.n_chunks - PARSE_AHEAD), dim3(64), 0, S, a->d_rfq, (uint64_t)a->n, D, B[DB_CHUNKS].as<DChunk>(), dst, PARSE_AHEAD);
            hipLaunchKernelGGL(k_dec_summary, dim3(1), dim3(256), 0, S, (const DChunk*)B[DB_CHUNKS].as<DChunk>(), dst, PARSE_AHEAD, hs.n_chunks - PARSE_AHEAD);
            KCHK(ctx, "k_dec_parse");
            DecStatus h2; HIPCHK(ctx, ctx->fetch(&h2, dst, sizeof h2, S));
            HIPCHK(ctx, ctx->fetch_sync(S));
            if (h2.pad) { guess = false; continue; }
            hs.max_stream = h2.max_stream; hs.max_npos = h2.max_npos; hs.max_len = h2.max_len; hs.max_bases = h2.max_bases; hs.max_nrec = h2.max_nrec;
                    hs.max_one = h2.max_one; hs.per_read_pieces = h2.per_read_pieces; hs.piece_avg = h2.piece_avg; hs.piece_n1 = h2.piece_n1;
                    memcpy(hs.base_slots, h2.base_slots, sizeof hs.base_slots);
        }
        if (hs.consumed != a->n && a->n - hs.consumed >= 18 && (a->final || hs.n_chunks == 0)) { guess = false; continue; }
        break;
    }
    if (ctx->opt.trace) fprintf(stderr, "[rfq] chunk starts: %s, %u chunks\n", use_table ? "caller's index" : (guess ? "guess-and-verify" : "exact walk"), hs.n_chunks);
    ctx->timer.end(S);
    if (hs.err & DE_CORRUPT) return rfq_fail(ctx, RFQ_E_FORMAT, "truncated or corrupt rfq chunk at byte %llu", (unsigned long long)hs.consumed);
    return RFQ_OK;
}

extern "C" int rfq_decode_batch(rfq_ctx* ctx, const rfq_decode_args* a, rfq_decode_result* res) {
    if (!ctx || !a || !res) return RFQ_E_ARG;
    memset(res, 0, sizeof *res);
    ctx->err.clear();
    if (a->n && !a->d_rfq) return rfq_fail(ctx, RFQ_E_ARG, "null rfq pointer");
    if (a->n == 0 && a->has_header) {
        if (a->split_pe) return rfq_fail(ctx, RFQ_E_DATA, "The input RFQ file was encoded by single-end FASTQ, you should not specify <out2>");
        return RFQ_OK;
    }
    uint64_t start = 0;
    { const int rc = dec_open(ctx, a, &start); if (rc) return rc; }
    const DevHeader& HH = ctx->h_hdr;
    if (a->split_pe && !(HH.flags & H_PAIRED)) return rfq_fail(ctx, RFQ_E_DATA, "The input RFQ file was encoded by single-end FASTQ, you should not specify <out2>");
    DecStatus hs;
    { const int rc = dec_walk(ctx, a, start, hs); if (rc) return rc; }
    DBuf* B = ctx->b; hipStream_t S = ctx->stream;
    uint64_t tb = 0; for (int i = 0; i < 16; i++) tb += hs.base_slots[i];
    const uint32_t n_chunks = hs.n_chunks; const uint64_t n_reads64 = hs.total_reads;
    res->consumed = (size_t)hs.consumed; res->n_chunks = n_chunks; res->n_reads = n_reads64;
    if (n_chunks == 0) return RFQ_OK;
    const uint32_t last_flags = hs.last_flags; const int split = a->split_pe ? 1 : 0;
    DChunk* CHm = B[DB_CHUNKS].as<DChunk>();
    const uint64_t slice_env = ctx->opt.slice_bases;
    const uint64_t slice_bases = slice_env ? slice_env : 1500000000ull, one_pass = slice_env ? slice_env : 0xFFFFFFF0ull;
    size_t n1 = 0, n2 = 0; uint64_t nb = 0; uint8_t *o1 = nullptr, *o2 = nullptr;
    int rc = RFQ_RANGE_TOO_BIG;
    std::vector<ChunkSpan> pieces; std::vector<DChunk> hc; bool strip1 = (last_flags & C_NO_LB) != 0, strip2 = (last_flags & C_NO_LB_R2) != 0;
    const bool compat = a->bug_compat != 0 && split;
    if (compat) {
        hc.resize(n_chunks);
        HIPCHK(ctx, hipMemcpy(hc.data(), CHm, (size_t)n_chunks * sizeof(DChunk), hipMemcpyDeviceToHost));
        uint32_t run = 0, end = n_chunks; strip1 = strip2 = false;
        for (uint32_t i = 0; i < n_chunks;) {
            const bool f1 = (hc[i].flags & C_NO_LB) != 0, f2 = split && (hc[i].flags & C_NO_LB_R2) != 0;
            if (!f1 && !f2) { i++; continue; }
            if (i + 1 == n_chunks) {
                if (!a->final) { end = i; res->consumed = (size_t)hc[i].off; }
                else { strip1 = f1; strip2 = f2; }
                break;
            }
            if (split && f1) { if (i > run) pieces.push_back({ run, i, false }); pieces.push_back({ i, i + 1, true }); }
            else pieces.push_back({ run, i + 1, false });
            run = i + 2; i += 2;
        }
        if (run < end) pieces.push_back({ run, end, false });
        res->n_chunks = 0; for (auto& q : pieces) res->n_chunks += q.c1 - q.c0;
    }
    if (!compat && tb < one_pass && n_reads64 < 0x7FFFFFF0ull) {
        const DecRange g = range_of(hs, CHm, n_chunks, n_reads64, tb);
        rc = decode_range(ctx, a, g, a->d_out1, a->cap1, a->d_out2, a->cap2, &o1, &o2, &n1, &n2, &nb);
        if (rc != RFQ_OK && rc != RFQ_RANGE_TOO_BIG) return rc;
    }
    if (rc == RFQ_RANGE_TOO_BIG) {
        if (!compat) { hc.resize(n_chunks); HIPCHK(ctx, hipMemcpy(hc.data(), CHm, (size_t)n_chunks * sizeof(DChunk), hipMemcpyDeviceToHost));
                pieces.push_back({ 0, n_chunks, false }); }
        std::vector<ChunkSpan> todo = plan_ranges(pieces, hc, slice_bases);
        size_t w1 = 0, w2 = 0; n1 = n2 = 0; nb = 0;
        StageSums sums; ctx->timer.collect(); sums.add(ctx->timer);
        while (!todo.empty()) {
            const ChunkSpan r = todo.back(); todo.pop_back();
            DecRange g; uint64_t reads = 0;
            rc = span_range(ctx, hs, CHm, hc, r, &g, &reads);
            if (rc) return rc;
            uint8_t *q1 = nullptr, *q2 = nullptr; size_t m1 = 0, m2 = 0; uint64_t mb = 0;
            ctx->timer.reset();
            rc = reads > 0x7FFFFFF0ull ? RFQ_RANGE_TOO_BIG : decode_range(ctx, a, g, nullptr, 0, nullptr, 0, &q1, &q2, &m1, &m2, &mb);
            if (rc == RFQ_RANGE_TOO_BIG) {
                if (r.c1 - r.c0 < 2) return rfq_fail(ctx, RFQ_E_ARG, "a single chunk decodes to 4 GiB of text or more");
                const uint32_t mid = r.c0 + (r.c1 - r.c0) / 2; todo.push_back({ mid, r.c1, r.r1_only }); todo.push_back({ r.c0, mid, r.r1_only }); continue;
            }
            if (rc != RFQ_OK) return rc;
            sums.add(ctx->timer);
            for (int k = 0; k < (split ? 2 : 1); k++) {
                uint8_t* src = k ? q2 : q1; const size_t m = k ? m2 : m1; size_t& w = k ? w2 : w1; uint8_t* dcall = k ? a->d_out2 : a->d_out1;
                        const size_t dcap = k ? a->cap2 : a->cap1;
                if (!m || (k && r.r1_only)) continue;
                uint8_t* to;
                if (dcall) { if (w + m > dcap) return rfq_fail(ctx, RFQ_E_NOSPACE, "output buffer too small"); to = dcall + w; }
                else { DBuf& ab = k ? ctx->out_acc2 : ctx->out_acc1; HIPCHK(ctx, ab.ensure_keep(w + m + 64, w, S)); to = ab.as<uint8_t>() + w; }
                HIPCHK(ctx, hipMemcpyAsync(to, src, m, hipMemcpyDeviceToDevice, S));
                w += m;
            }
            HIPCHK(ctx, hipStreamSynchronize(S));
            nb += mb;
        }
        n1 = w1; n2 = w2;
        o1 = a->d_out1 ? a->d_out1 : ctx->out_acc1.as<uint8_t>(); o2 = a->d_out2 ? a->d_out2 : ctx->out_acc2.as<uint8_t>();
        sums.publish(ctx->timer);
    }
    res->n_bases = nb;
    if (a->final) {
        if (strip1 && n1) n1--;
        if (split && strip2 && n2) n2--;
    }
    res->d_fq1 = o1; res->n1 = n1; res->d_fq2 = split ? o2 : nullptr; res->n2 = split ? n2 : 0;
    return RFQ_OK;
}

static int rows_range(rfq_ctx* ctx, const rfq_decode_args* a, const DecRange& g, const RowsOut& o) {
    hipStream_t S = ctx->stream; DBuf* B = ctx->b; const DevHeader* D = ctx->d_hdr.as<DevHeader>(); DecStatus* dst = B[DB_STATUS].as<DecStatus>();
    HIPCHK(ctx, hipMemsetAsync(dst, 0, sizeof(DecStatus), S));
    ctx->timer.begin("read_table", S);
    const size_t nr = (size_t)g.n_reads + 2;
    HIPCHK(ctx, B[DB_LEN].ensure(nr * 4)); HIPCHK(ctx, B[DB_OV].ensure(nr * 4));
    DReadTab R; memset(&R, 0, sizeof R); R.len = B[DB_LEN].as<uint32_t>(); R.ov = B[DB_OV].as<int32_t>();
    uint32_t total_bases = 0; U4 pv_tot; memset(&pv_tot, 0, sizeof pv_tot);
    int rc = dec_table_expanded(ctx, a, g, R, false, &total_bases, &pv_tot);
    if (rc) return rc;
    DecExpanded E; rc = dec_streams_expanded(ctx, a, g, R, total_bases, pv_tot, false, &E);
    if (rc) return rc;
    DecStatus h; HIPCHK(ctx, ctx->fetch(&h, dst, sizeof h, S)); HIPCHK(ctx, ctx->fetch_sync(S));
    if (h.err & DE_CORRUPT) return rfq_fail(ctx, RFQ_E_FORMAT, "corrupt quality buffer");
    ctx->timer.begin("rows", S);
    const uint32_t bx = grid_x_for(g.n_chunks, (std::max(g.max_reads, 1u) + 31u) / 32u, 8u * ctx->n_cu);
    hipLaunchKernelGGL(k_dec_rows, dim3(bx, g.n_chunks), dim3(256), 0, S, g.CH, (const DevHeader*)D, R, (const uint64_t*)E.qbase, (const uint64_t*)E.sbase,
                       (const uint8_t*)E.qdec, (const uint8_t*)E.sdec, o);
    KCHK(ctx, "k_dec_rows");
    ctx->timer.end(S);
    HIPCHK(ctx, hipStreamSynchronize(S));
    return RFQ_OK;
}

extern "C" int rfq_decode_rows(rfq_ctx* ctx, const rfq_decode_rows_args* ra, rfq_decode_rows_result* res) {
    if (!ctx || !ra || !res) return RFQ_E_ARG;
    memset(res, 0, sizeof *res);
    ctx->err.clear();
    if (ra->n && !ra->d_rfq) return rfq_fail(ctx, RFQ_E_ARG, "null rfq pointer");
    if (ra->base_mode != RFQ_ROWS_ASCII && ra->base_mode != RFQ_ROWS_CODE) return rfq_fail(ctx, RFQ_E_ARG, "base_mode must be RFQ_ROWS_ASCII or RFQ_ROWS_CODE");
    const bool query = !ra->d_bases && !ra->d_quals && !ra->d_lens;
    if (!query && ra->row_len == 0) return rfq_fail(ctx, RFQ_E_ARG, "row_len must be at least 1");
    if ((uintptr_t)ra->d_lens & 3u) return rfq_fail(ctx, RFQ_E_ARG, "d_lens must be 4-byte aligned");
    rfq_decode_args a; memset(&a, 0, sizeof a);
    a.d_rfq = ra->d_rfq; a.n = ra->n; a.has_header = ra->has_header; a.final = ra->final; a.h_chunk_off = ra->h_chunk_off; a.n_chunk_off = ra->n_chunk_off;
    if (a.n == 0 && a.has_header) return RFQ_OK;
    uint64_t start = 0;
    { const int rc = dec_open(ctx, &a, &start); if (rc) return rc; }
    DecStatus hs;
    { const int rc = dec_walk(ctx, &a, start, hs); if (rc) return rc; }
    hipStream_t S = ctx->stream;
    uint64_t tb = 0; for (int i = 0; i < 16; i++) tb += hs.base_slots[i];
    const uint32_t n_chunks = hs.n_chunks; const uint64_t n_rows = n_chunks ? hs.total_reads : 0;
    res->consumed = (size_t)hs.consumed; res->n_chunks = n_chunks; res->n_rows = n_rows; res->n_bases = n_chunks ? tb : 0; res->max_len = n_chunks ? hs.max_len : 0;
    if (query || n_chunks == 0) { HIPCHK(ctx, hipStreamSynchronize(S)); ctx->timer.collect(); return RFQ_OK; }
    const uint64_t L = ra->row_len, need = n_rows * L;
    if (L < res->max_len) return rfq_fail(ctx, RFQ_E_NOSPACE, "row_len %u is shorter than the longest read: need row_len >= %u", ra->row_len, res->max_len);
    if (ra->d_bases && ra->bases_cap < need) return rfq_fail(ctx, RFQ_E_NOSPACE, "base rows too small: need %llu bytes (%llu rows of %u)", (unsigned long long)need,
            (unsigned long long)n_rows, ra->row_len);
    if (ra->d_quals && ra->quals_cap < need) return rfq_fail(ctx, RFQ_E_NOSPACE, "quality rows too small: need %llu bytes (%llu rows of %u)", (unsigned long long)need,
            (unsigned long long)n_rows, ra->row_len);
    if (ra->d_lens && ra->lens_cap < n_rows) return rfq_fail(ctx, RFQ_E_NOSPACE, "length array too small: need %llu entries", (unsigned long long)n_rows);
    RowsOut o; memset(&o, 0, sizeof o);
    o.bases = ra->d_bases; o.quals = ra->d_quals; o.lens = ra->d_lens; o.row_len = L; o.n_rows = n_rows;
    o.codes = ra->base_mode == RFQ_ROWS_CODE ? 1u : 0u;
    o.qoff4 = ra->qual_offset * 0x01010101u; o.pad_b4 = ra->pad_base * 0x01010101u; o.pad_q4 = ra->pad_qual * 0x01010101u;
    o.vec = (L % 16u == 0 && !((uintptr_t)ra->d_bases & 15u) && !((uintptr_t)ra->d_quals & 15u)) ? 1u : 0u;
    DChunk* CHm = ctx->b[DB_CHUNKS].as<DChunk>();
    const uint64_t slice_env = ctx->opt.slice_bases;
    const uint64_t slice_bases = slice_env ? slice_env : 1500000000ull, one_pass = slice_env ? slice_env : 0xFFFFFFF0ull;
    if (tb < one_pass && n_rows < 0x7FFFFFF0ull) {
        const int rc = rows_range(ctx, &a, range_of(hs, CHm, n_chunks, n_rows, tb), o);
        if (rc) return rc;
        ctx->timer.collect();
        return RFQ_OK;
    }
    std::vector<DChunk> hc(n_chunks);
    HIPCHK(ctx, hipMemcpy(hc.data(), CHm, (size_t)n_chunks * sizeof(DChunk), hipMemcpyDeviceToHost));
    std::vector<ChunkSpan> todo = plan_ranges(std::vector<ChunkSpan>{ { 0, n_chunks, false } }, hc, slice_bases);
    HIPCHK(ctx, hipStreamSynchronize(S));
    StageSums sums; ctx->timer.collect(); sums.add(ctx->timer);
    while (!todo.empty()) {
        const ChunkSpan r = todo.back(); todo.pop_back();
        DecRange g; uint64_t reads = 0;
        int rc = span_range(ctx, hs, CHm, hc, r, &g, &reads);
        if (rc) return rc;
        if (g.bases >= 0xFFFFFFF0ull || reads >= 0x7FFFFFF0ull) return rfq_fail(ctx, RFQ_E_ARG, "a single chunk holds 4 Gi bases or 2 Gi reads or more");
        ctx->timer.reset();
        rc = rows_range(ctx, &a, g, o);
        if (rc) return rc;
        ctx->timer.collect(); sums.add(ctx->timer);
    }
    sums.publish(ctx->timer);
    return RFQ_OK;
}
```

Measured before the change: 1.100 million MB/s.

## Fuse position-list sum, link, offset and list kernels into one LDS-staged kernel

Replaces the four-kernel chain for building per-stream position lists (segment sum, wave link scan, global offset prefix, list emit) with one kernel per (stream, chunk) block. The block stages the stream bytes in LDS, keeps the segment tables in LDS, and assigns list offsets with an atomicAdd on list_need instead of a separate prefix kernel. This removes launches and global round trips for the segment tables and reads each stream from LDS twice rather than from global memory. In exchange, list order in the output buffer becomes nondeterministic, large LDS allocations may lower occupancy, and streams that do not fit in LDS fall back to the alias/retry path.

```diff
diff --git a/repaq_amd/csrc/dec/pos_lists.h b/repaq_amd/csrc/dec/pos_lists.h
--- a/repaq_amd/csrc/dec/pos_lists.h
+++ b/repaq_amd/csrc/dec/pos_lists.h
@@ -56,6 +56,28 @@
 }
 #define POS_ADV_MAX 0x3FFFFFFFull
 __device__ __forceinline__ int pos_adv_sat(int v) { return v > (int)POS_ADV_MAX ? (int)POS_ADV_MAX : v; }
+template <class Fetch> __device__ __forceinline__ void pos_seg_sum(const PosSrc& s, uint32_t b0, uint32_t b1, Fetch fetch, uint32_t& Fcum, int (&a)[4], int (&n)[4]) {
+    const int l = lane_id();
+    Fcum = POS_ID;
+#pragma unroll
+    for (int e = 0; e < 4; e++) { a[e] = 0; n[e] = 0; }
+    PosStep nxt = fetch(b0 + 4u * (uint32_t)l);
+    for (uint32_t base = b0; base < b1; base += 256u) {
+        const uint32_t i0 = base + 4u * (uint32_t)l;
+        const PosStep w = nxt;
+        if (base + 256u < b1) nxt = fetch(i0 + 256u);
+        const PosFront f = pos_front(w, s.sp, s.slen, i0, l);
+        const uint32_t Fex = wave_shr1(f.Fin, POS_ID);
+        const uint32_t G = fn_compose(Fcum, Fex);
+        int la[4], lc[4]; pos_lane_adv_cnt4(f, s.slen, i0, la, lc);
+#pragma unroll
+        for (int e = 0; e < 4; e++) { const uint32_t t_ = fn_apply(G, e); a[e] += sel4(la, t_); n[e] += sel4(lc, t_); }
+        Fcum = fn_compose(Fcum, wave_last(f.Fin));
+    }
+#pragma unroll
+    for (int e = 0; e < 4; e++) { const unsigned long long w64 = wave_sum<unsigned long long>((unsigned long long)(uint32_t)a[e]); a[e] = (int)(w64 > POS_ADV_MAX ? POS_ADV_MAX : w64);
+            n[e] = wave_sum(n[e]); }
+}
 __global__ void k_dec_pos_sum2(const uint8_t* __restrict__ img, const DChunk* __restrict__ CH, const DevHeader* __restrict__ D,
                                uint8_t* __restrict__ segF, int* __restrict__ segA, uint32_t* __restrict__ segN, uint32_t maxseg, DecStatus* st, uint64_t img_bytes, uint32_t jj0, uint32_t nstr,
                                uint32_t segb) {
@@ -66,23 +88,8 @@
     if (g == 0 && l == 0) segN[(size_t)c * nstr + jj] = (s.slen + segb - 1) / segb;
     const uint32_t b0 = g * segb; if (b0 >= s.slen) return;
     const uint32_t b1 = b0 + segb < s.slen ? b0 + segb : s.slen;
-    uint32_t Fcum = POS_ID; int a[4] = { 0, 0, 0, 0 }, n[4] = { 0, 0, 0, 0 };
-    PosStep nxt = pos_fetch(s.sp, s.slen, b0 + 4u * (uint32_t)l, lim);
-    for (uint32_t base = b0; base < b1; base += 256u) {
-        const uint32_t i0 = base + 4u * (uint32_t)l;
-        const PosStep w = nxt;
-        if (base + 256u < b1) nxt = pos_fetch(s.sp, s.slen, i0 + 256u, lim);
-        const PosFront f = pos_front(w, s.sp, s.slen, i0, l);
-        const uint32_t Fex = wave_shr1(f.Fin, POS_ID);
-        const uint32_t G = fn_compose(Fcum, Fex);
-        int la[4], lc[4]; pos_lane_adv_cnt4(f, s.slen, i0, la, lc);
-#pragma unroll
-        for (int e = 0; e < 4; e++) { const uint32_t t_ = fn_apply(G, e); a[e] += sel4(la, t_); n[e] += sel4(lc, t_); }
-        Fcum = fn_compose(Fcum, wave_last(f.Fin));
-    }
-#pragma unroll
-    for (int e = 0; e < 4; e++) { const unsigned long long w64 = wave_sum<unsigned long long>((unsigned long long)(uint32_t)a[e]); a[e] = (int)(w64 > POS_ADV_MAX ? POS_ADV_MAX : w64);
-            n[e] = wave_sum(n[e]); }
+    uint32_t Fcum; int a[4], n[4];
+    pos_seg_sum(s, b0, b1, [&](uint32_t i0) { return pos_fetch(s.sp, s.slen, i0, lim); }, Fcum, a, n);
     if (l == 0) { const size_t idx = ((size_t)c * nstr + jj) * maxseg + g; segF[idx] = (uint8_t)fn_pack8(Fcum);
 #pragma unroll
                   for (int e = 0; e < 4; e++) { segA[8 * idx + e] = a[e]; segA[8 * idx + 4 + e] = n[e]; } }
@@ -100,38 +107,44 @@
     for (int s = 0; s < 4; s++) { u.a[s] = __shfl_up(v.a[s], dd); u.n[s] = __shfl_up(v.n[s], dd); }
     return u;
 }
+template <class Load, class Store> __device__ __forceinline__ void pos_link_scan(uint32_t n, Load load, Store store, int& cp, uint32_t& ck) {
+    const int l = lane_id();
+    uint32_t cs = 0; cp = -1; ck = 0;
+    for (uint32_t base = 0; base < n; base += 64) {
+        const uint32_t g = base + (uint32_t)l;
+        PosLink me; me.F = POS_ID;
+#pragma unroll
+        for (int s = 0; s < 4; s++) { me.a[s] = 0; me.n[s] = 0; }
+        if (g < n) me = load(g);
+        PosLink inc = me;
+#pragma unroll
+        for (int dd = 1; dd < 64; dd <<= 1) { const PosLink up = poslink_shfl_up(inc, (unsigned)dd); if (l >= dd) inc = poslink_then(up, inc); }
+        PosLink ex = poslink_shfl_up(inc, 1u);
+        if (l == 0) { ex.F = POS_ID;
+#pragma unroll
+                      for (int s = 0; s < 4; s++) { ex.a[s] = 0; ex.n[s] = 0; } }
+        if (g < n) store(g, fn_apply(ex.F, cs), pos_adv_sat(cp + sel4(ex.a, cs)), ck + (uint32_t)sel4(ex.n, cs));
+        const uint32_t Fl = wave_last(inc.F); int al[4], nl[4];
+#pragma unroll
+        for (int s = 0; s < 4; s++) { al[s] = wave_last(inc.a[s]); nl[s] = wave_last(inc.n[s]); }
+        cp = pos_adv_sat(cp + sel4(al, cs)); ck += (uint32_t)sel4(nl, cs); cs = fn_apply(Fl, cs);
+    }
+}
+__device__ __forceinline__ bool pos_list_aliases(int cp, unsigned long long chunk_bases) { return cp >= 0 && (unsigned long long)cp >= chunk_bases + 32768ull; }
 __global__ void k_dec_pos_link2(const uint8_t* __restrict__ segF, const int* __restrict__ segA, const uint32_t* __restrict__ segN, uint8_t* __restrict__ segS,
         int* __restrict__ segP,
                                 uint32_t* __restrict__ segK, uint32_t* __restrict__ nent, uint32_t maxseg, uint32_t n_streams,
                                 const DChunk* __restrict__ CH, uint32_t nstr, DecStatus* st) {
     const uint32_t t = blockIdx.x * (blockDim.x >> 6) + (uint32_t)wave_id(); if (t >= n_streams) return;
-    const int l = lane_id(); const uint32_t n = segN[t];
-    uint32_t cs = 0; int cp = -1; uint32_t ck = 0;
-    for (uint32_t base = 0; base < n; base += 64) {
-        const uint32_t g = base + (uint32_t)l; const size_t idx = (size_t)t * maxseg + g;
-        PosLink me; me.F = POS_ID;
-#pragma unroll
-        for (int s = 0; s < 4; s++) { me.a[s] = 0; me.n[s] = 0; }
-        if (g < n) { me.F = fn_unpack8(segF[idx]);
-#pragma unroll
-                     for (int s = 0; s < 4; s++) { me.a[s] = segA[8 * idx + s]; me.n[s] = segA[8 * idx + 4 + s]; } }
-        PosLink inc = me;
-#pragma unroll
-        for (int dd = 1; dd < 64; dd <<= 1) { const PosLink up = poslink_shfl_up(inc, (unsigned)dd); if (l >= dd) inc = poslink_then(up, inc); }
-        PosLink ex = poslink_shfl_up(inc, 1u);
-        if (l == 0) { ex.F = POS_ID;
-#pragma unroll
-                      for (int s = 0; s < 4; s++) { ex.a[s] = 0; ex.n[s] = 0; } }
-        if (g < n) { segS[idx] = (uint8_t)(fn_apply(ex.F, cs)); segP[idx] = pos_adv_sat(cp + sel4(ex.a, cs)); segK[idx] = ck + (uint32_t)sel4(ex.n, cs); }
-        const uint32_t Fl = wave_last(inc.F); int al[4], nl[4];
-#pragma unroll
-        for (int s = 0; s < 4; s++) { al[s] = wave_last(inc.a[s]); nl[s] = wave_last(inc.n[s]); }
-        cp = pos_adv_sat(cp + sel4(al, cs)); ck += (uint32_t)sel4(nl, cs); cs = fn_apply(Fl, cs);
-    }
-    if (l == 0) {
+    const size_t i0 = (size_t)t * maxseg; int cp; uint32_t ck;
+    pos_link_scan(segN[t],
+        [&](uint32_t g) { const size_t idx = i0 + g; PosLink me; me.F = fn_unpack8(segF[idx]);
+                          for (int s = 0; s < 4; s++) { me.a[s] = segA[8 * idx + s]; me.n[s] = segA[8 * idx + 4 + s]; }
+                          return me; },
+        [&](uint32_t g, uint32_t S, int P, uint32_t K) { const size_t idx = i0 + g; segS[idx] = (uint8_t)S; segP[idx] = P; segK[idx] = K; }, cp, ck);
+    if (lane_id() == 0) {
         nent[t] = ck;
-        const unsigned long long ext = CH[t / nstr].bases;
-        if (cp >= 0 && (unsigned long long)cp >= ext + 32768ull) atomicOr(&st->err, (uint32_t)DE_LIST_ALIAS);
+        if (pos_list_aliases(cp, CH[t / nstr].bases)) atomicOr(&st->err, (uint32_t)DE_LIST_ALIAS);
     }
 }
 __global__ void k_dec_pos_off(const uint32_t* __restrict__ nent, unsigned long long* __restrict__ loff, uint32_t n_streams, DecStatus* st) {
@@ -142,25 +155,14 @@
     for (uint32_t i = i0; i < i1; i++) { loff[i] = run; run += nent[i]; }
     if (threadIdx.x == 0) st->list_need = tot;
 }
-__global__ void k_dec_pos_list(const uint8_t* __restrict__ img, const DChunk* __restrict__ CH, const DevHeader* __restrict__ D,
-                               const uint8_t* __restrict__ segS, const int* __restrict__ segP, const uint32_t* __restrict__ segK, const unsigned long long* __restrict__ loff,
-                               plist_t* __restrict__ plist, unsigned long long cap, uint32_t* __restrict__ cellidx, uint32_t maxseg, uint32_t ncell, uint64_t img_bytes, uint32_t jj0, uint32_t nstr, const DecStatus* st,
-                               uint32_t segb) {
-    if (st->list_need > cap) return;
-    const uint32_t g = blockIdx.x * (blockDim.x >> 6) + (uint32_t)wave_id(), jj = jj0 + blockIdx.y, c = blockIdx.z; const int l = lane_id();
-            const uint8_t* lim = img + img_bytes;
-    const DChunk d = CH[c];
-    const PosSrc s = pos_src_of(img, d, D, jj, nullptr);
-    const uint32_t b0 = g * segb; if (b0 >= s.slen) return;
-    const size_t t = (size_t)c * nstr + jj, idx = t * maxseg + g;
-    uint32_t carry = segS[idx]; int last = segP[idx]; uint32_t k0 = segK[idx];
-    plist_t* const out = plist + loff[t]; uint32_t* const cells = cellidx + t * ncell;
-    const uint32_t b1 = b0 + segb < s.slen ? b0 + segb : s.slen;
-    PosStep nxt = pos_fetch(s.sp, s.slen, b0 + 4u * (uint32_t)l, lim);
+template <class Fetch> __device__ __forceinline__ void pos_seg_list(const PosSrc& s, uint32_t b0, uint32_t b1, Fetch fetch, uint32_t carry, int last, uint32_t k0,
+                                                                    plist_t* __restrict__ out, uint32_t* __restrict__ cells, uint32_t ncell) {
+    const int l = lane_id();
+    PosStep nxt = fetch(b0 + 4u * (uint32_t)l);
     for (uint32_t base = b0; base < b1; base += 256u) {
         const uint32_t i0 = base + 4u * (uint32_t)l;
         const PosStep w = nxt;
-        if (base + 256u < b1) nxt = pos_fetch(s.sp, s.slen, i0 + 256u, lim);
+        if (base + 256u < b1) nxt = fetch(i0 + 256u);
         const PosFront f = pos_front(w, s.sp, s.slen, i0, l);
         const uint32_t Fex = wave_shr1(f.Fin, POS_ID);
         uint32_t st0 = fn_apply(Fex, carry);
@@ -196,6 +198,92 @@
             }
         }
         last += wave_last(ia); k0 += (uint32_t)wave_last(ic); carry = fn_apply((uint32_t)wave_last(f.Fin), carry);
+    }
+}
+__global__ void k_dec_pos_list(const uint8_t* __restrict__ img, const DChunk* __restrict__ CH, const DevHeader* __restrict__ D,
+                               const uint8_t* __restrict__ segS, const int* __restrict__ segP, const uint32_t* __restrict__ segK, const unsigned long long* __restrict__ loff,
+                               plist_t* __restrict__ plist, unsigned long long cap, uint32_t* __restrict__ cellidx, uint32_t maxseg, uint32_t ncell, uint64_t img_bytes, uint32_t jj0, uint32_t nstr, const DecStatus* st,
+                               uint32_t segb) {
+    if (st->list_need > cap) return;
+    const uint32_t g = blockIdx.x * (blockDim.x >> 6) + (uint32_t)wave_id(), jj = jj0 + blockIdx.y, c = blockIdx.z;
+            const uint8_t* lim = img + img_bytes;
+    const DChunk d = CH[c];
+    const PosSrc s = pos_src_of(img, d, D, jj, nullptr);
+    const uint32_t b0 = g * segb; if (b0 >= s.slen) return;
+    const size_t t = (size_t)c * nstr + jj, idx = t * maxseg + g;
+    const uint32_t b1 = b0 + segb < s.slen ? b0 + segb : s.slen;
+    pos_seg_list(s, b0, b1, [&](uint32_t i0) { return pos_fetch(s.sp, s.slen, i0, lim); }, segS[idx], segP[idx], segK[idx], plist + loff[t], cellidx + t * ncell, ncell);
+}
+#define POS2_FUSED_SEG_LDS 48u
+#define POS2_FUSED_LDS_MAX (160u * 1024u)
+#define POS2_FUSED_STAGE_MAX (159u * 1024u)
+#define POS2_FUSED_WAVES 16u
+__device__ __host__ __forceinline__ uint32_t pos_fused_lbytes(uint32_t max_stream) { return (max_stream + 15u + 32u + 15u) & ~15u; }
+__global__ void __launch_bounds__(1024) k_dec_pos_fused(const uint8_t* __restrict__ img, const DChunk* __restrict__ CH, const DevHeader* __restrict__ D, uint32_t* __restrict__ nent,
+                                unsigned long long* __restrict__ loff, plist_t* __restrict__ plist, unsigned long long cap, uint32_t* __restrict__ cellidx, uint32_t ncell,
+                                uint32_t maxseg, uint32_t lbytes, uint64_t img_bytes, uint32_t nn, uint32_t nstr, uint32_t segb, DecStatus* st) {
+    RFQ_DYN_SHARED(uint4, s_dyn);
+    __shared__ unsigned long long s_off;
+    uint8_t* const lb = (uint8_t*)s_dyn;
+    uint32_t* const sF = (uint32_t*)(lb + lbytes); int* const sA = (int*)(sF + maxseg);
+    uint32_t* const sS = (uint32_t*)(sA + 8 * maxseg); int* const sP = (int*)(sS + maxseg); uint32_t* const sK = (uint32_t*)(sP + maxseg);
+    const uint32_t c = blockIdx.y, jj = blockIdx.x < nn ? blockIdx.x : D->n_normal, tid = threadIdx.x, w = (uint32_t)wave_id(), nw = blockDim.x >> 6; const int l = lane_id();
+    const uint8_t* lim = img + img_bytes;
+    const DChunk d = CH[c];
+    const PosSrc s = pos_src_of(img, d, D, jj, w == 0 ? st : nullptr);
+    const size_t t = (size_t)c * nstr + jj;
+    const uint32_t sh = (uint32_t)((uintptr_t)s.sp & 15u), nseg = (s.slen + segb - 1) / segb;
+    const bool fits = (!lbytes || (uint64_t)sh + s.slen + 32u <= lbytes) && nseg <= maxseg;
+    if (s.slen == 0 || !fits) {
+        if (tid == 0) { nent[t] = 0; loff[t] = 0; if (s.slen) atomicOr(&st->err, (uint32_t)DE_LIST_ALIAS); }
+        return;
+    }
+    const uint8_t* const g0 = s.sp - sh; const uint32_t ngr = (sh + s.slen + 15u) / 16u;
+    for (uint32_t q = tid; lbytes && q <= ngr; q += blockDim.x) {
+        const uint8_t* p = g0 + 16u * (size_t)q; uint4 v = make_uint4(0u, 0u, 0u, 0u);
+        if (q < ngr) {
+            if (p >= img && p + 16 <= lim) v = *(const uint4*)p;
+            else { uint32_t x[4] = { 0u, 0u, 0u, 0u };
+                   for (int k = 0; k < 16; k++) if (p + k >= img && p + k < lim) x[k >> 2] |= (uint32_t)p[k] << (8 * (k & 3));
+                   v = make_uint4(x[0], x[1], x[2], x[3]); }
+        }
+        s_dyn[q] = v;
+    }
+    __syncthreads();
+    auto fetch = [&](uint32_t i0) { if (!lbytes) return pos_fetch(s.sp, s.slen, i0, lim);
+                                    PosStep r; r.w0 = r.w1 = r.w2 = 0;
+                                    if (i0 < s.slen) { const uint32_t* p = (const uint32_t*)(lb + ((sh + i0) & ~3u)); r.w0 = p[0]; r.w1 = p[1]; r.w2 = p[2]; }
+                                    return r; };
+    for (uint32_t g = w; g < nseg; g += nw) {
+        const uint32_t b0 = g * segb, b1 = b0 + segb < s.slen ? b0 + segb : s.slen;
+        uint32_t Fcum; int a[4], n[4];
+        pos_seg_sum(s, b0, b1, fetch, Fcum, a, n);
+        if (l == 0) { sF[g] = Fcum;
+#pragma unroll
+                      for (int e = 0; e < 4; e++) { sA[8 * g + e] = a[e]; sA[8 * g + 4 + e] = n[e]; } }
+    }
+    __syncthreads();
+    if (w == 0) {
+        int cp; uint32_t ck;
+        pos_link_scan(nseg,
+            [&](uint32_t g) { PosLink me; me.F = sF[g];
+                              for (int e = 0; e < 4; e++) { me.a[e] = sA[8 * g + e]; me.n[e] = sA[8 * g + 4 + e]; }
+                              return me; },
+            [&](uint32_t g, uint32_t S, int P, uint32_t K) { sS[g] = S; sP[g] = P; sK[g] = K; }, cp, ck);
+        if (l == 0) {
+            if (pos_list_aliases(cp, d.bases)) atomicOr(&st->err, (uint32_t)DE_LIST_ALIAS);
+            const unsigned long long off = ck ? atomicAdd(&st->list_need, (unsigned long long)ck) : 0ull;
+            nent[t] = ck; loff[t] = off;
+            s_off = off + ck <= cap ? off : ~0ull;
+        }
+    }
+    __syncthreads();
+    const unsigned long long off = s_off;
+    if (off == ~0ull) return;
+    plist_t* const out = plist + off; uint32_t* const cells = cellidx + t * ncell;
+    for (uint32_t g = w; g < nseg; g += nw) {
+        const uint32_t b0 = g * segb, b1 = b0 + segb < s.slen ? b0 + segb : s.slen;
+        pos_seg_list(s, b0, b1, fetch, sS[g], sP[g], sK[g], out, cells, ncell);
     }
 }
 
diff --git a/repaq_amd/csrc/rfq_api.hip b/repaq_amd/csrc/rfq_api.hip
--- a/repaq_amd/csrc/rfq_api.hip
+++ b/repaq_amd/csrc/rfq_api.hip
@@ -42,11 +42,15 @@
     else if (n == "RFQ_SP_PAD") { RFQ_OPT_NUM(0, 150000, "0 .. 150000 bytes of LDS") c->opt.sp_pad = set ? (uint32_t)num : d.sp_pad; }
     else if (n == "RFQ_POS_SEG") { if (set && v != "1024" && v != "2048") return rfq_fail(c, RFQ_E_ARG, "RFQ_POS_SEG is 1024 or 2048"); c->opt.pos_seg = set ? atoi(v.c_str()) : 0; }
     else if (n == "RFQ_SPEC") { if (set && v != "0" && v != "1") return rfq_fail(c, RFQ_E_ARG, "RFQ_SPEC is 0 or 1"); c->opt.no_spec = v == "0"; }
+    else if (n == "RFQ_LISTS") { if (set && v != "fused" && v != "chain") return rfq_fail(c, RFQ_E_ARG, "RFQ_LISTS is fused or chain");
+            c->opt.lists = v == "fused" ? 1 : (v == "chain" ? 2 : 0); }
+    else if (n == "RFQ_POS_LDS") { RFQ_OPT_NUM(256, 163840, "256 .. 163840 bytes of LDS") c->opt.pos_lds = set ? (uint32_t)num : 0u; }
+    else if (n == "RFQ_POS_WAVES") { RFQ_OPT_NUM(1, 16, "1 .. 16") c->opt.pos_waves = set ? (int)num : 0; }
     else return rfq_fail(c, RFQ_E_ARG, "unknown option %s", name);
 #undef RFQ_OPT_NUM
     return RFQ_OK;
 }
-static const char* const RFQ_OPTION_NAMES[] = { "RFQ_GATHER", "RFQ_QUAL", "RFQ_CODER", "RFQ_INDEX", "RFQ_IDX_TILES", "RFQ_STREAMS", "RFQ_SLICE_BYTES", "RFQ_SLICE_BASES", "RFQ_WALK", "RFQ_GW_SHIFT", "RFQ_MATERIALISE", "RFQ_TRACE", "RFQ_G2_PAD", "RFQ_SP_PAD", "RFQ_POS_SEG", "RFQ_SPEC" };
+static const char* const RFQ_OPTION_NAMES[] = { "RFQ_GATHER", "RFQ_QUAL", "RFQ_CODER", "RFQ_INDEX", "RFQ_IDX_TILES", "RFQ_STREAMS", "RFQ_SLICE_BYTES", "RFQ_SLICE_BASES", "RFQ_WALK", "RFQ_GW_SHIFT", "RFQ_MATERIALISE", "RFQ_TRACE", "RFQ_G2_PAD", "RFQ_SP_PAD", "RFQ_POS_SEG", "RFQ_SPEC", "RFQ_LISTS", "RFQ_POS_LDS", "RFQ_POS_WAVES" };
 extern "C" const char* rfq_option_name(int i) { return (i >= 0 && i < (int)(sizeof RFQ_OPTION_NAMES / sizeof RFQ_OPTION_NAMES[0])) ? RFQ_OPTION_NAMES[i] : nullptr; }
 extern "C" int rfq_get_option(const rfq_ctx* c, const char* name, char* out, size_t cap) {
     if (!c || !name || !out || !cap) return RFQ_E_ARG;
@@ -67,6 +71,9 @@
     else if (n == "RFQ_SP_PAD") v = o.sp_pad != d.sp_pad ? std::to_string(o.sp_pad) : "";
     else if (n == "RFQ_POS_SEG") v = o.pos_seg ? std::to_string(o.pos_seg) : "";
     else if (n == "RFQ_SPEC") v = o.no_spec ? "0" : "";
+    else if (n == "RFQ_LISTS") v = o.lists == 1 ? "fused" : (o.lists == 2 ? "chain" : "");
+    else if (n == "RFQ_POS_LDS") v = o.pos_lds ? std::to_string(o.pos_lds) : "";
+    else if (n == "RFQ_POS_WAVES") v = o.pos_waves ? std::to_string(o.pos_waves) : "";
     else return RFQ_E_ARG;
     if (v.size() + 1 > cap) return RFQ_E_NOSPACE;
     memcpy(out, v.c_str(), v.size() + 1);
diff --git a/repaq_amd/csrc/rfq_ctx.h b/repaq_amd/csrc/rfq_ctx.h
--- a/repaq_amd/csrc/rfq_ctx.h
+++ b/repaq_amd/csrc/rfq_ctx.h
@@ -86,9 +86,13 @@
     uint32_t sp_pad = 0;
     bool no_spec = false;
     int  pos_seg = 0;
+    int  lists = 0;
+    uint32_t pos_lds = 0;
+    int  pos_waves = 0;
 };
 struct rfq_ctx {
     RfqOpts opt;
+    uint32_t pos_fused_lds = 65536;
     bool e3_pieces_failed = false;
     int device = 0; uint32_t n_cu = 256;
     hipStream_t stream = nullptr; bool own_stream = false;
diff --git a/repaq_amd/csrc/rfq_decode.hip b/repaq_amd/csrc/rfq_decode.hip
--- a/repaq_amd/csrc/rfq_decode.hip
+++ b/repaq_amd/csrc/rfq_decode.hip
@@ -104,17 +104,50 @@
     const bool on = !force_expanded && !ctx->opt.materialise && !rle_h && g.max_len <= 2000u && g.max_nrec <= 4096u && e3_ok && g.max_bases < (1u << 30) - 65536u;
     return { on, e3k, n1big, E3_SHARED_OK && !g.pieces && !(HH.flags & H_DONT_QUAL) };
 }
-struct ListChain { uint32_t maxseg = 1, ncell = 1, nstr = 1, mq = 0, mn = 0, nn = 0, segb = POS2_SEG; bool hasn = false, built = false, join = false; hipStream_t aux = nullptr; };
+struct ListChain { uint32_t maxseg = 1, ncell = 1, nstr = 1, mq = 0, mn = 0, nn = 0, segb = POS2_SEG; bool hasn = false, built = false, join = false; hipStream_t aux = nullptr;
+        bool fused = false; uint32_t lbytes = 0, lds = 0, threads = 64; };
 struct AuxJoin { rfq_ctx* c; bool armed; ~AuxJoin() { if (armed) (void)hipStreamSynchronize(c->aux); } };
 
-static void launch_pos_list(rfq_ctx* ctx, const rfq_decode_args* a, const DecRange& g, const ListChain& L, hipStream_t LS) {
-    DBuf* B = ctx->b; const DevHeader* D = ctx->d_hdr.as<DevHeader>(); const DecStatus* dst = B[DB_STATUS].as<DecStatus>();
+static hipError_t launch_pos_list(rfq_ctx* ctx, const rfq_decode_args* a, const DecRange& g, const ListChain& L, hipStream_t LS, bool again) {
+    DBuf* B = ctx->b; const DevHeader* D = ctx->d_hdr.as<DevHeader>(); DecStatus* dst = B[DB_STATUS].as<DecStatus>();
     const unsigned long long cap = B[DB_PLIST].cap / sizeof(plist_t);
+    if (L.fused) {
+        if (again) { const hipError_t e = hipMemsetAsync(&dst->list_need, 0, sizeof dst->list_need, LS); if (e != hipSuccess) return e; }
+        hipLaunchKernelGGL(k_dec_pos_fused, dim3(L.nn + (L.hasn ? 1u : 0u), g.n_chunks), dim3(L.threads), L.lds, LS, a->d_rfq, g.CH, D, B[DB_NENT].as<uint32_t>(),
+                           B[DB_LOFF].as<unsigned long long>(), B[DB_PLIST].as<plist_t>(), cap, B[DB_CELL].as<uint32_t>(), L.ncell, L.maxseg, L.lbytes, (uint64_t)a->n,
+                           L.nn, L.nstr, L.segb, dst);
+        return hipSuccess;
+    }
 #define RFQ_LIST_ARGS a->d_rfq, g.CH, D, (const uint8_t*)B[DB_SEGS].as<uint8_t>(), (const int*)B[DB_SEGP].as<int>(), (const uint32_t*)B[DB_SEGK].as<uint32_t>(), \
                       (const unsigned long long*)B[DB_LOFF].as<unsigned long long>(), B[DB_PLIST].as<plist_t>(), cap, B[DB_CELL].as<uint32_t>(), L.maxseg, L.ncell, (uint64_t)a->n
     if (L.nn) hipLaunchKernelGGL(k_dec_pos_list, dim3((L.mq + 3) / 4, L.nn, g.n_chunks), dim3(256), 0, LS, RFQ_LIST_ARGS, 0u, L.nstr, dst, L.segb);
     if (L.hasn) hipLaunchKernelGGL(k_dec_pos_list, dim3((L.mn + 3) / 4, 1, g.n_chunks), dim3(256), 0, LS, RFQ_LIST_ARGS, ctx->h_hdr.n_normal, L.nstr, dst, L.segb);
 #undef RFQ_LIST_ARGS
+    return hipSuccess;
+}
+static bool plan_pos_fused(rfq_ctx* ctx, const DecRange& g, ListChain* L) {
+    if (ctx->opt.lists == 2) return false;
+    const uint32_t maxlen = std::max(L->nn ? g.max_one : 0u, L->hasn ? g.max_npos : 0u), segb = ctx->opt.pos_seg ? (uint32_t)ctx->opt.pos_seg : POS2_SEG;
+    const uint32_t maxseg = maxlen / segb + 1, tables = POS2_FUSED_SEG_LDS * maxseg;
+#ifdef RFQ_SIMT_EMULATION
+    const uint32_t room = 65536u;
+#else
+    const uint32_t room = POS2_FUSED_LDS_MAX - 1024u;
+#endif
+    if (tables > room / 2) return false;
+    const uint32_t budget = ctx->opt.pos_lds ? std::min(ctx->opt.pos_lds, room) : std::min(POS2_FUSED_STAGE_MAX, room);
+    uint32_t lbytes = maxlen <= POS2_FUSED_LDS_MAX ? pos_fused_lbytes(maxlen) : 0u;
+    if (!lbytes || lbytes + tables > budget) lbytes = 0;
+    const uint32_t lds = lbytes + tables;
+#ifndef RFQ_SIMT_EMULATION
+    if (lds > ctx->pos_fused_lds) {
+        if (hipFuncSetAttribute((const void*)k_dec_pos_fused, hipFuncAttributeMaxDynamicSharedMemorySize, (int)room) != hipSuccess) { (void)hipGetLastError(); return false; }
+        ctx->pos_fused_lds = room;
+    }
+#endif
+    const uint32_t waves = ctx->opt.pos_waves ? (uint32_t)ctx->opt.pos_waves : POS2_FUSED_WAVES;
+    L->fused = true; L->segb = segb; L->maxseg = maxseg; L->lbytes = lbytes; L->lds = lds; L->threads = 64u * std::min(waves, maxseg);
+    return true;
 }
 static int dec_list_chain(rfq_ctx* ctx, const rfq_decode_args* a, const DecRange& g, AuxJoin& guard, ListChain* L) {
     hipStream_t S = ctx->stream; DBuf* B = ctx->b; const DevHeader& HH = ctx->h_hdr; const DevHeader* D = ctx->d_hdr.as<DevHeader>();
@@ -124,17 +157,28 @@
     if (!L->nn && !L->hasn) return RFQ_OK;
     const bool forked = ctx->aux_ready(); hipStream_t A = forked ? ctx->aux : S;
     if (forked) { HIPCHK(ctx, hipEventRecord(ctx->ev_fork, S)); HIPCHK(ctx, hipStreamWaitEvent(A, ctx->ev_fork, 0)); guard.armed = true; }
-    L->segb = ctx->opt.pos_seg ? (uint32_t)ctx->opt.pos_seg : (std::max(g.max_one, g.max_npos) >= 32768u ? POS2_SEG_BIG : POS2_SEG);
-    L->mq = L->nn ? g.max_one / L->segb + 1 : 0u; L->mn = L->hasn ? g.max_npos / L->segb + 1 : 0u; L->maxseg = std::max(1u, std::max(L->mq, L->mn));
+    if (!plan_pos_fused(ctx, g, L)) {
+        L->segb = ctx->opt.pos_seg ? (uint32_t)ctx->opt.pos_seg : (std::max(g.max_one, g.max_npos) >= 32768u ? POS2_SEG_BIG : POS2_SEG);
+        L->mq = L->nn ? g.max_one / L->segb + 1 : 0u; L->mn = L->hasn ? g.max_npos / L->segb + 1 : 0u; L->maxseg = std::max(1u, std::max(L->mq, L->mn));
+    }
     L->ncell = g.max_bases / POS2_CELL + 2;
     const size_t nst = (size_t)n_chunks * L->nstr, nseg = nst * L->maxseg, ncl = nst * L->ncell;
-    HIPCHK(ctx, B[DB_SEGF].ensure(nseg + 16)); HIPCHK(ctx, B[DB_SEGA].ensure(nseg * 32 + 16)); HIPCHK(ctx, B[DB_SEGN].ensure(nst * 4 + 16));
-    HIPCHK(ctx, B[DB_SEGS].ensure(nseg + 16)); HIPCHK(ctx, B[DB_SEGP].ensure(nseg * 4 + 16)); HIPCHK(ctx, B[DB_SEGK].ensure(nseg * 4 + 16));
+    if (!L->fused) {
+        HIPCHK(ctx, B[DB_SEGF].ensure(nseg + 16)); HIPCHK(ctx, B[DB_SEGA].ensure(nseg * 32 + 16)); HIPCHK(ctx, B[DB_SEGN].ensure(nst * 4 + 16));
+        HIPCHK(ctx, B[DB_SEGS].ensure(nseg + 16)); HIPCHK(ctx, B[DB_SEGP].ensure(nseg * 4 + 16)); HIPCHK(ctx, B[DB_SEGK].ensure(nseg * 4 + 16));
+    }
     HIPCHK(ctx, B[DB_CELL].ensure(ncl * 4 + 16));
     HIPCHK(ctx, B[DB_NENT].ensure(nst * 4 + 16)); HIPCHK(ctx, B[DB_LOFF].ensure(nst * 8 + 16));
     if (B[DB_PLIST].ensure((size_t)(g.bases / 8 + 1024) * sizeof(plist_t)) != hipSuccess) { (void)hipGetLastError();
             HIPCHK(ctx, B[DB_PLIST].ensure((size_t)(g.bases / 32 + 1024) * sizeof(plist_t))); }
-    { ClearList z; memset(&z, 0, sizeof z); z.add(B[DB_SEGN].p, nst * 4, 0u); z.add(B[DB_NENT].p, nst * 4, 0u); z.add(B[DB_CELL].p, ncl * 4, 0xFFFFFFFFu); clear_list(A, z); }
+    { ClearList z; memset(&z, 0, sizeof z); if (!L->fused) z.add(B[DB_SEGN].p, nst * 4, 0u); z.add(B[DB_NENT].p, nst * 4, 0u); z.add(B[DB_CELL].p, ncl * 4, 0xFFFFFFFFu);
+      clear_list(A, z); }
+    if (L->fused) {
+        HIPCHK(ctx, launch_pos_list(ctx, a, g, *L, A, false));
+        L->built = true; L->join = forked; L->aux = A;
+        KCHK(ctx, "k_dec_pos_fused");
+        return RFQ_OK;
+    }
 #define RFQ_SUM2_ARGS a->d_rfq, CH, D, B[DB_SEGF].as<uint8_t>(), B[DB_SEGA].as<int>(), B[DB_SEGN].as<uint32_t>(), L->maxseg, dst, (uint64_t)a->n
     if (L->nn) hipLaunchKernelGGL(k_dec_pos_sum2, dim3((L->mq + 3) / 4, L->nn, n_chunks), dim3(256), 0, A, RFQ_SUM2_ARGS, 0u, L->nstr, L->segb);
     if (L->hasn) hipLaunchKernelGGL(k_dec_pos_sum2, dim3((L->mn + 3) / 4, 1, n_chunks), dim3(256), 0, A, RFQ_SUM2_ARGS, HH.n_normal, L->nstr, L->segb);
@@ -143,7 +187,7 @@
                        (const uint32_t*)B[DB_SEGN].as<uint32_t>(), B[DB_SEGS].as<uint8_t>(), B[DB_SEGP].as<int>(), B[DB_SEGK].as<uint32_t>(), B[DB_NENT].as<uint32_t>(),
                        L->maxseg, (uint32_t)nst, CH, L->nstr, dst);
     hipLaunchKernelGGL(k_dec_pos_off, dim3(1), dim3(256), 0, A, (const uint32_t*)B[DB_NENT].as<uint32_t>(), B[DB_LOFF].as<unsigned long long>(), (uint32_t)nst, dst);
-    launch_pos_list(ctx, a, g, *L, A);
+    HIPCHK(ctx, launch_pos_list(ctx, a, g, *L, A, false));
     L->built = true; L->join = forked; L->aux = A;
     KCHK(ctx, "k_dec_pos_*");
     return RFQ_OK;
@@ -250,7 +294,7 @@
         if (L.built && hs.list_need > B[DB_PLIST].cap / sizeof(plist_t)) {
             if (emitted) { emitted = false; ctx->timer.begin("streams", S); }
             HIPCHK(ctx, B[DB_PLIST].ensure((size_t)(hs.list_need + 1024) * sizeof(plist_t)));
-            launch_pos_list(ctx, a, g, L, S);
+            HIPCHK(ctx, launch_pos_list(ctx, a, g, L, S, true));
             KCHK(ctx, "k_dec_pos_list");
         }
         hs.text1 = hs.text2 = 0; for (int i = 0; i < 64; i++) { hs.text1 += hs.text_slots[0][i]; hs.text2 += hs.text_slots[1][i]; }
```

Result: slower. 1.069 million MB/s (-2.7%).
